# irconde/SSL4POLYP

Hardware: AMD Instinct MI355X
Metric: training-step images/sec/node, ViT-B/16 224^2 (cls fine-tune) (higher is better)
Workload: dtype bf16; 1 GPU; ViT-B/16 classification fine-tune, bs=64/GPU, 224^2, AdamW, random init, finetune mode full (finetune.py:49-91); global_batch=64, parallelism=dp1, launch=eager, lr_schedule=constant

## Files before the change

include/polypmae.h:

```cpp
#ifndef POLYPMAE_H
#define POLYPMAE_H
#include <stddef.h>
#include <stdint.h>

#ifdef __cplusplus
extern "C" {
#endif

enum pm_status { PM_OK = 0, PM_EINVAL = -1, PM_ESHAPE = -2, PM_EARCH = -3, PM_ELAUNCH = -4, PM_EALIGN = -5 };
enum pm_dtype { PM_F32 = 0, PM_BF16 = 1, PM_F16 = 2 };

enum pm_epilogue {
  PM_EPI_STORE = 0,
  PM_EPI_GELU = 1,
  PM_EPI_RESIDUAL = 2,
  PM_EPI_DGELU = 3,
  PM_EPI_ACCUM = 4
};

const char* pm_strerror(int status);
int pm_abi_version(void);

int pm_layernorm_fwd(const float* x, long ldx, const float* gamma, const float* beta, void* y, int out_dtype,
                     float* mean, float* rstd, int M, int D, float eps, void* stream);

int pm_layernorm_bwd(const void* dy, int dy_dtype, const float* x, long ldx, const float* gamma, const float* mean,
                     const float* rstd, const float* dres, long lddres, float* dx, long lddx, void* dx_act,
                     int act_dtype, float* dgamma, float* dbeta, float* dcolsum, int M, int D, void* workspace,
                     size_t ws_bytes, void* stream);

int pm_gemm(const void* A, long lda, int a_kmajor, const void* B, long ldb, int b_kmajor, int in_dtype,
            const float* bias, void* C, long ldc, int c_dtype, int epilogue, void* aux, const float* resid,
            int M, int N, int K, void* stream);

int pm_gemm_ws(const void* A, long lda, int a_kmajor, const void* B, long ldb, int b_kmajor, int in_dtype,
               const float* bias, void* C, long ldc, int c_dtype, int epilogue, void* aux, const float* resid,
               int M, int N, int K, void* workspace, size_t ws_bytes, void* stream);

typedef struct pm_gemm_opts {
  int max_blocks;
  int variant;
} pm_gemm_opts;
int pm_gemm_ex(const void* A, long lda, int a_kmajor, const void* B, long ldb, int b_kmajor, int in_dtype,
               const float* bias, void* C, long ldc, int c_dtype, int epilogue, void* aux, const float* resid,
               int M, int N, int K, void* workspace, size_t ws_bytes, const pm_gemm_opts* opts, void* stream);

typedef struct pm_wgrad_item {
  const void* dY;
  long lddy;
  const void* X;
  long ldx;
  float* dW;
  long lddw;
  int n_out, n_in;
  int accumulate;
  float* dbias;
} pm_wgrad_item;
#define PM_GROUP_WHOLE_K (-1)
int pm_wgrad_group(const pm_wgrad_item* items, int n, int K, int in_dtype, int max_blocks, void* workspace, size_t ws_bytes,
                   void* stream);
size_t pm_wgrad_group_workspace_bytes(const pm_wgrad_item* items, int n, int K, int in_dtype);
int pm_wgrad_group_plan(const pm_wgrad_item* items, int n, int K, int in_dtype, size_t* ws_bytes, int* tiles256,
                        int* k_slices);

int pm_gemm_colsum(const void* A, long lda, int a_kmajor, const void* B, long ldb, int b_kmajor, int in_dtype,
                   const float* bias, void* C, long ldc, int c_dtype, int epilogue, void* aux, const float* resid,
                   float* colsum, int M, int N, int K, void* workspace, size_t ws_bytes, void* stream);

int pm_attention_fwd(const void* qkv, void* out, float* lse, int B, int N, int H, int dh, int dtype, void* stream);
int pm_attention_bwd(const void* qkv, const void* out, const void* dout, const float* lse, float* delta, void* dqkv,
                     int B, int N, int H, int dh, int dtype, void* stream);

int pm_colsum(const void* x, long ldx, int dtype, float* out, int M, int N, void* stream);
int pm_colsum_ws(const void* x, long ldx, int dtype, float* out, int M, int N, void* workspace, size_t ws_bytes,
                 void* stream);

int pm_patch_im2col(const float* imgs, const int* ids_keep, void* cols, long ldcols, int out_dtype, int B, int C, int img,
                    int p, int keep, void* stream);

int pm_pad_cast(const float* src, long lds, void* dst, long ldd, int dst_dtype, int rows, int cols, int rows_pad,
                int cols_pad, void* stream);
int pm_unpad_add(const float* src, long lds, float* dst, long ldd, int rows, int cols, int accumulate, void* stream);

int pm_assemble_tokens(const float* emb, const float* cls, const float* pos, const int* ids_keep, float* x,
                       int B, int keep, int D, void* stream);
int pm_assemble_tokens_bwd(const float* dx, const int* ids_keep, void* demb, int act_dtype, float* dcls, float* dpos,
                           int B, int keep, int D, void* stream);

int pm_mae_noise(float* noise, long n, unsigned long long seed, unsigned int stream_id, void* stream);
int pm_mae_masking(const float* noise, int* ids_shuffle, int* ids_restore, float* mask, int B, int L, int len_keep,
                   void* stream);

int pm_mae_unshuffle(const float* emb, const float* mask_token, const float* dpos, const int* ids_restore, float* out,
                     int B, int L, int keep, int D, void* stream);
int pm_mae_unshuffle_bwd(const float* dout, const int* ids_shuffle, void* demb, int act_dtype, float* dmask_token,
                         int B, int L, int keep, int D, void* workspace, size_t ws_bytes, void* stream);

int pm_mae_loss_fwd(const float* imgs, const float* pred, long ldp, int has_cls_row, float* patch_loss, int B, int C,
                    int img, int p, int norm_pix, void* stream);
int pm_mae_loss_finish(const float* patch_loss, const float* mask, long n, float* sums, float* loss, void* stream);
int pm_mae_loss_bwd(const float* imgs, const float* pred, long ldp, int has_cls_row, const float* mask,
                    const float* sums, const float* dloss, void* dpred, long lddp, int act_dtype, int B, int C, int img,
                    int p, int norm_pix, void* stream);

int pm_gather_rows(const void* src, long ld_bytes, const int* idx, void* dst, int R, long row_bytes, void* stream);
int pm_scatter_rows_zero(const void* src, const int* inv, void* dst, int M, long row_bytes, void* stream);

int pm_cast(const float* src, void* dst, int dst_dtype, long n, void* stream);

int pm_preprocess_u8(const unsigned char* src, const unsigned char* flip_flags, float* dst, int B, int H, int W,
                     float mean_r, float mean_g, float mean_b, float std_r, float std_g, float std_b, void* stream);


int pm_aug_resize_u8(const unsigned char* src, unsigned char* tmp, unsigned char* dst, const int* bounds_x, const int* taps_x,
                     int ksize_x, const int* bounds_y, const int* taps_y, int ksize_y, int B, int Hs, int Ws, int Ho, int Wo,
                     void* stream);

size_t pm_aug_resized_crop_workspace_bytes(int B, int Hs, int Ws, int out);
int pm_aug_resized_crop_u8(const unsigned char* src, const int* box, unsigned char* dst, int bicubic, int B, int Hs, int Ws, int out,
                           void* workspace, size_t ws_bytes, void* stream);
int pm_aug_resized_crop_ragged_u8(const unsigned char* src, const long long* offset, const int* hw, const int* box, unsigned char* dst,
                                  int bicubic, int B, int Hmax, int Wmax, int out, void* workspace, size_t ws_bytes, void* stream);

typedef struct pm_aug_jitter {
  int order[4];
  float brightness, contrast, saturation;
  int hue_shift;
} pm_aug_jitter;
int pm_aug_color_jitter_u8(const unsigned char* src, unsigned char* dst, const pm_aug_jitter* jitter, unsigned long long* lsum,
                           int B, int H, int W, void* stream);

int pm_aug_gaussian_blur_u8(const unsigned char* src, float* tmp, unsigned char* dst, const float* taps, int ksize, int B, int H,
                            int W, void* stream);

typedef struct pm_aug_geom {
  int mode, a0, a1, a2, a3, a4, a5, flips;
} pm_aug_geom;
int pm_aug_geometry_u8(const unsigned char* src, const pm_aug_geom* geom, void* dst, int to_f32, int B, int H, int W, float mean_r,
                       float mean_g, float mean_b, float std_r, float std_g, float std_b, void* stream);

typedef struct pm_aug_boxblur {
  int radius;
  unsigned int ww, fw;
} pm_aug_boxblur;
int pm_aug_pil_gaussian_blur_u8(const unsigned char* src, unsigned char* tmp, unsigned char* dst, const pm_aug_boxblur* prm,
                                int passes, int B, int H, int W, void* stream);
int pm_aug_occlude_u8(unsigned char* img, const int* rects, int B, int H, int W, void* stream);
int pm_aug_jpeg_roundtrip_u8(const unsigned char* src, unsigned char* dst, const int* quality, int B, int H, int W, void* stream);

int pm_jpeg_decode(const unsigned char* entropy, long entropy_bytes, const int* intervals, int n_intervals, const int* frames,
                   int n_frames, const unsigned char* huff, int n_huff, const int* quant, int n_quant, const unsigned char* fallback,
                   long fallback_bytes, const long long* fallback_table, int n_fallback, short* coef, unsigned char* planes,
                   long blocks, long pixels, unsigned char* out, long out_bytes, void* stream);

int pm_jpeg_decode_workspace(int n_intervals, int n_subseq, size_t* bytes);
int pm_jpeg_decode_parallel(const unsigned char* entropy, long entropy_bytes, const int* intervals, int n_intervals, const int* frames,
                            int n_frames, const unsigned char* huff, int n_huff, const int* quant, int n_quant,
                            const unsigned char* fallback, long fallback_bytes, const long long* fallback_table, int n_fallback,
                            short* coef, unsigned char* planes, long blocks, long pixels, unsigned char* out, long out_bytes,
                            const int* subseq, int n_subseq, int sync_rounds, void* workspace, size_t ws_bytes, int* stats,
                            void* stream);

int pm_jpeg_decode_planes(const unsigned char* entropy, long entropy_bytes, const int* intervals, int n_intervals, const int* frames,
                          int n_frames, const unsigned char* huff, int n_huff, const int* quant, int n_quant, short* coef,
                          unsigned char* planes, long blocks, const int* subseq, int n_subseq, int sync_rounds, void* workspace,
                          size_t ws_bytes, int* stats, void* stream);

int pm_jpeg_resized_crop_workspace(int B, int Hmax, int Wmax, int out, size_t* bytes);
int pm_jpeg_resized_crop_u8(const unsigned char* planes, long blocks, const int* frames, int n_frames, const unsigned char* fallback,
                            long fallback_bytes, const long long* fallback_table, int n_fallback, const int* source, const int* hw,
                            const int* box, unsigned char* dst, int bicubic, int B, int Hmax, int Wmax, int out, void* workspace,
                            size_t ws_bytes, void* stream);

typedef struct pm_block_fwd_desc {
  const float* x;
  float* x_mid;
  float* x_out;
  void* ln1;
  float* mean1;
  float* rstd1;
  void* qkv;
  float* lse;
  void* attn;
  void* ln2;
  float* mean2;
  float* rstd2;
  void* h_pre;
  void* h_act;
  const float *norm1_w, *norm1_b, *norm2_w, *norm2_b;
  const void *qkv_w, *proj_w, *fc1_w, *fc2_w;
  const float *qkv_b, *proj_b, *fc1_b, *fc2_b;
  int rows, samples, N, D, Hd, heads;
  int dtype;
  int gemm_variant;
  float eps;
} pm_block_fwd_desc;
int pm_vit_block_fwd(const pm_block_fwd_desc* d, void* stream);

typedef struct pm_block_bwd_desc {
  const float* x_in;
  const float* x_mid;
  const void *ln1, *qkv, *attn, *ln2, *h_pre, *h_act;
  const float *mean1, *rstd1, *mean2, *rstd2, *lse;
  const float *norm1_w, *norm2_w;
  const void *qkv_w, *proj_w, *fc1_w, *fc2_w;
  const float* dx;
  const void* dx_act;
  float* dmid;
  void* dmid_act;
  float* din;
  void* din_act;
  void *d_hidden, *d_qkv, *d_ln, *d_attn;
  float* delta;
  float *g_norm1_w, *g_norm1_b, *g_norm2_w, *g_norm2_b;
  float *g_qkv_w, *g_proj_w, *g_fc1_w, *g_fc2_w;
  float *g_qkv_b, *g_proj_b, *g_fc1_b, *g_below_bias;
  void* ws_ln;
  size_t ws_ln_bytes;
  void* ws_group;
  size_t ws_group_bytes;
  void *side_stream, *ev_join, *ev_fork, *ev_done;
  int samples, N, D, Hd, heads, dtype, gemm_variant, group_blocks, accumulate;
  int two_groups;
  void *side_stream2, *ev_fork2, *ev_done2;
} pm_block_bwd_desc;
int pm_vit_block_bwd(const pm_block_bwd_desc* d, void* stream);

int pm_vit_head_fwd(const float* x, int N, int pool, const float* gamma, const float* beta, const float* W,
                    const float* bias, float* feat, float* xhat_mean, float* mean, float* rstd, float* logits, int B, int D,
                    int n_class, float eps, void* stream);
int pm_vit_head_bwd(const float* dlogits, const float* dfeat, const float* x, int N, int pool, const float* gamma,
                    const float* W, const float* feat, const float* xhat_mean, const float* mean, const float* rstd,
                    float* dx, void* dx_act, int act_dtype, float* dW, float* dbias, float* dgamma, float* dbeta, int B,
                    int D, int n_class, void* stream);
int pm_cls_head_fwd(const float* x, int N, const float* gamma, const float* beta, const float* W, const float* bias,
                    float* xn, float* mean, float* rstd, float* logits, int B, int D, int n_class, float eps,
                    void* stream);
int pm_cls_head_bwd(const float* dlogits, const float* x, int N, const float* gamma, const float* W, const float* xn,
                    const float* mean, const float* rstd, float* dx, void* dx_act, int act_dtype, float* dW,
                    float* dbias, float* dgamma, float* dbeta, int B, int D, int n_class, void* stream);

int pm_supervised_loss_fwd(const float* logits, const long long* targets, const float* pos_weight,
                           const float* class_weights, float* loss, float* dlogits, int B, int n_class, void* stream);
int pm_scale(const float* x, const float* scale, float* out, long n, void* stream);

int pm_dgelu(const void* dy, const void* pre, void* out, int dtype, long n, void* stream);

int pm_adamw(float* p, const float* g, float* m, float* v, void* shadow, int shadow_dtype, long n, float lr,
             float beta1, float beta2, float eps, float weight_decay, int step, float grad_scale, void* stream);

int pm_adamw_tick(float* hyper, int n_groups, void* stream);
int pm_adamw_dev(float* p, const float* g, float* m, float* v, void* shadow, int shadow_dtype, long n,
                 const float* hyper, void* stream);

int pm_loss_scale_update(float* state, const float* stats, float* hyper, int n_groups, float growth_factor,
                         float backoff_factor, int growth_interval, void* stream);

int pm_grad_stats(const float* g, long n, float* out, void* stream);

enum pm_ws_kind { PM_WS_LAYERNORM_BWD = 1, PM_WS_COLSUM = 2, PM_WS_GEMM_COLSUM = 3, PM_WS_UNSHUFFLE_BWD = 4 };
size_t pm_gemm_workspace_bytes(int a_kmajor, int b_kmajor, int in_dtype, int M, int N, int K, const pm_gemm_opts* opts);
size_t pm_workspace_bytes(int kind, int M, int N);

typedef struct pm_comm pm_comm;
int pm_comm_unique_id(void* id128);
int pm_comm_create(pm_comm** out, const void* id128, int rank, int world);
int pm_comm_world(const pm_comm* c, int* rank, int* world);
int pm_comm_allreduce_f32(pm_comm* c, float* base, const long* lo, const long* hi, int n_buckets, void* stream);
int pm_comm_destroy(pm_comm* c);

int pm_boot_metrics_workspace(int N, int M, int R, int K, int C, size_t* bytes);
int pm_boot_metrics(const double* score, const int* order, const unsigned char* label, const int* cluster, const int* draws,
                    const double* tau, double* out, int N, int M, int R, int K, int C, int sorted_ready, void* workspace,
                    size_t ws_bytes, void* stream);

#ifdef __cplusplus
}
#endif
#endif
```

ssl4polyp_amd/_lib.py:

```python
from __future__ import annotations

import ctypes
import os
from ctypes import c_char_p, c_float, c_int, c_long, c_void_p

PM_F32, PM_BF16, PM_F16 = 0, 1, 2
EPI_STORE, EPI_GELU, EPI_RESIDUAL, EPI_DGELU, EPI_ACCUM = 0, 1, 2, 3, 4

_HERE = os.path.dirname(os.path.abspath(__file__))
LIB_PATH = os.environ.get("POLYPMAE_LIB") or os.path.join(_HERE, "lib", "libpolypmae.so")

P, I, L, F = c_void_p, c_int, c_long, c_float

SIGNATURES = {
    "pm_layernorm_fwd": [P, L, P, P, P, I, P, P, I, I, F, P],
    "pm_layernorm_bwd": [P, I, P, L, P, P, P, P, L, P, L, P, I, P, P, P, I, I, P, ctypes.c_size_t, P],
    "pm_vit_block_fwd": [P, P],
    "pm_vit_block_bwd": [P, P],
    "pm_gemm": [P, L, I, P, L, I, I, P, P, L, I, I, P, P, I, I, I, P],
    "pm_gemm_ws": [P, L, I, P, L, I, I, P, P, L, I, I, P, P, I, I, I, P, ctypes.c_size_t, P],
    "pm_gemm_ex": [P, L, I, P, L, I, I, P, P, L, I, I, P, P, I, I, I, P, ctypes.c_size_t, P, P],
    "pm_wgrad_group": [P, I, I, I, I, P, ctypes.c_size_t, P],
    "pm_wgrad_group_plan": [P, I, I, I, P, P, P],
    "pm_gemm_colsum": [P, L, I, P, L, I, I, P, P, L, I, I, P, P, P, I, I, I, P, ctypes.c_size_t, P],
    "pm_attention_fwd": [P, P, P, I, I, I, I, I, P],
    "pm_attention_bwd": [P, P, P, P, P, P, I, I, I, I, I, P],
    "pm_colsum": [P, L, I, P, I, I, P],
    "pm_colsum_ws": [P, L, I, P, I, I, P, ctypes.c_size_t, P],
    "pm_patch_im2col": [P, P, P, L, I, I, I, I, I, I, P],
    "pm_pad_cast": [P, L, P, L, I, I, I, I, I, P],
    "pm_unpad_add": [P, L, P, L, I, I, I, P],
    "pm_assemble_tokens": [P, P, P, P, P, I, I, I, P],
    "pm_assemble_tokens_bwd": [P, P, P, I, P, P, I, I, I, P],
    "pm_mae_noise": [P, L, ctypes.c_ulonglong, ctypes.c_uint, P],
    "pm_mae_masking": [P, P, P, P, I, I, I, P],
    "pm_mae_unshuffle": [P, P, P, P, P, I, I, I, I, P],
    "pm_mae_unshuffle_bwd": [P, P, P, I, P, I, I, I, I, P, ctypes.c_size_t, P],
    "pm_mae_loss_fwd": [P, P, L, I, P, I, I, I, I, I, P],
    "pm_mae_loss_finish": [P, P, L, P, P, P],
    "pm_mae_loss_bwd": [P, P, L, I, P, P, P, P, L, I, I, I, I, I, I, P],
    "pm_cast": [P, P, I, L, P],
    "pm_gather_rows": [P, L, P, P, I, L, P],
    "pm_scatter_rows_zero": [P, P, P, I, L, P],
    "pm_preprocess_u8": [P, P, P, I, I, I, F, F, F, F, F, F, P],
    "pm_aug_resize_u8": [P, P, P, P, P, I, P, P, I, I, I, I, I, I, P],
    "pm_aug_resized_crop_u8": [P, P, P, I, I, I, I, I, P, ctypes.c_size_t, P],
    "pm_aug_resized_crop_ragged_u8": [P, P, P, P, P, I, I, I, I, I, P, ctypes.c_size_t, P],
    "pm_aug_color_jitter_u8": [P, P, P, P, I, I, I, P],
    "pm_aug_gaussian_blur_u8": [P, P, P, P, I, I, I, I, P],
    "pm_aug_geometry_u8": [P, P, P, I, I, I, I, F, F, F, F, F, F, P],
    "pm_aug_pil_gaussian_blur_u8": [P, P, P, P, I, I, I, I, P],
    "pm_aug_occlude_u8": [P, P, I, I, I, P],
    "pm_aug_jpeg_roundtrip_u8": [P, P, P, I, I, I, P],
    "pm_jpeg_decode": [P, L, P, I, P, I, P, I, P, I, P, L, P, I, P, P, L, L, P, L, P],
    "pm_jpeg_decode_parallel": [P, L, P, I, P, I, P, I, P, I, P, L, P, I, P, P, L, L, P, L, P, I, I, P, ctypes.c_size_t, P, P],
    "pm_jpeg_decode_workspace": [I, I, P],
    "pm_jpeg_decode_planes": [P, L, P, I, P, I, P, I, P, I, P, P, L, P, I, I, P, ctypes.c_size_t, P, P],
    "pm_jpeg_resized_crop_workspace": [I, I, I, I, P],
    "pm_jpeg_resized_crop_u8": [P, L, P, I, P, L, P, I, P, P, P, P, I, I, I, I, I, P, ctypes.c_size_t, P],
    "pm_comm_unique_id": [P],
    "pm_comm_create": [P, P, I, I],
    "pm_comm_world": [P, P, P],
    "pm_comm_allreduce_f32": [P, P, P, P, I, P],
    "pm_comm_destroy": [P],
    "pm_vit_head_fwd": [P, I, I, P, P, P, P, P, P, P, P, P, I, I, I, F, P],
    "pm_vit_head_bwd": [P, P, P, I, I, P, P, P, P, P, P, P, P, I, P, P, P, P, I, I, I, P],
    "pm_supervised_loss_fwd": [P, P, P, P, P, P, I, I, P],
    "pm_scale": [P, P, P, L, P],
    "pm_cls_head_fwd": [P, I, P, P, P, P, P, P, P, P, I, I, I, F, P],
    "pm_cls_head_bwd": [P, P, I, P, P, P, P, P, P, P, I, P, P, P, P, I, I, I, P],
    "pm_adamw": [P, P, P, P, P, I, L, F, F, F, F, F, I, F, P],
    "pm_adamw_tick": [P, I, P],
    "pm_adamw_dev": [P, P, P, P, P, I, L, P, P],
    "pm_grad_stats": [P, L, P, P],
    "pm_loss_scale_update": [P, P, P, I, F, F, I, P],
    "pm_dgelu": [P, P, P, I, L, P],
    "pm_boot_metrics_workspace": [I, I, I, I, I, P],
    "pm_boot_metrics": [P, P, P, P, P, P, P, I, I, I, I, I, I, P, ctypes.c_size_t, P],
}

ABI_VERSION = 14
PM_GROUP_WHOLE_K = -1

WS_LAYERNORM_BWD, WS_COLSUM, WS_GEMM_COLSUM, WS_UNSHUFFLE_BWD = 1, 2, 3, 4


class GemmOpts(ctypes.Structure):
    _fields_ = [("max_blocks", c_int), ("variant", c_int)]


class WgradItem(ctypes.Structure):
    _fields_ = [("dY", c_void_p), ("lddy", c_long), ("X", c_void_p), ("ldx", c_long), ("dW", c_void_p), ("lddw", c_long),
                ("n_out", c_int), ("n_in", c_int), ("accumulate", c_int), ("dbias", c_void_p)]


class BlockBwdDesc(ctypes.Structure):
    _fields_ = ([(n, c_void_p) for n in ("x_in", "x_mid", "ln1", "qkv", "attn", "ln2", "h_pre", "h_act", "mean1", "rstd1", "mean2",
                                        "rstd2", "lse", "norm1_w", "norm2_w", "qkv_w", "proj_w", "fc1_w", "fc2_w", "dx", "dx_act",
                                        "dmid", "dmid_act", "din", "din_act", "d_hidden", "d_qkv", "d_ln", "d_attn", "delta",
                                        "g_norm1_w", "g_norm1_b", "g_norm2_w", "g_norm2_b", "g_qkv_w", "g_proj_w", "g_fc1_w",
                                        "g_fc2_w", "g_qkv_b", "g_proj_b", "g_fc1_b", "g_below_bias")] +
                [("ws_ln", c_void_p), ("ws_ln_bytes", ctypes.c_size_t), ("ws_group", c_void_p), ("ws_group_bytes", ctypes.c_size_t)] +
                [(n, c_void_p) for n in ("side_stream", "ev_join", "ev_fork", "ev_done")] +
                [(n, c_int) for n in ("samples", "N", "D", "Hd", "heads", "dtype", "gemm_variant", "group_blocks", "accumulate",
                                      "two_groups")] +
                [(n, c_void_p) for n in ("side_stream2", "ev_fork2", "ev_done2")])


class BlockFwdDesc(ctypes.Structure):
    _fields_ = ([(n, c_void_p) for n in ("x", "x_mid", "x_out", "ln1", "mean1", "rstd1", "qkv", "lse", "attn", "ln2", "mean2",
                                        "rstd2", "h_pre", "h_act", "norm1_w", "norm1_b", "norm2_w", "norm2_b", "qkv_w", "proj_w",
                                        "fc1_w", "fc2_w", "qkv_b", "proj_b", "fc1_b", "fc2_b")] +
                [(n, c_int) for n in ("rows", "samples", "N", "D", "Hd", "heads", "dtype", "gemm_variant")] +
                [("eps", ctypes.c_float)])


PM_EINVAL, PM_ESHAPE, PM_EALIGN = -1, -2, -5
_lib = None


class PolypMaeError(RuntimeError):
    pass


def load():
    global _lib
    if _lib is not None:
        return _lib
    if not os.path.exists(LIB_PATH):
        raise PolypMaeError(
            f"{LIB_PATH} not found: build it with `python -c 'import __graft_entry__ as g; g.build()'`. "
            "There is no CPU/eager fallback for the MI355X hot path.")
    lib = ctypes.CDLL(LIB_PATH)
    lib.pm_strerror.restype = c_char_p
    lib.pm_strerror.argtypes = [c_int]
    lib.pm_abi_version.restype = c_int
    lib.pm_abi_version.argtypes = []
    if lib.pm_abi_version() != ABI_VERSION:
        raise PolypMaeError(f"{LIB_PATH} has ABI version {lib.pm_abi_version()}, this package binds version {ABI_VERSION}: "
                            "rebuild with `python -c 'import __graft_entry__ as g; g.build(force=True)'`")
    lib.pm_gemm_workspace_bytes.restype = ctypes.c_size_t
    lib.pm_gemm_workspace_bytes.argtypes = [I, I, I, I, I, I, P]
    lib.pm_workspace_bytes.restype = ctypes.c_size_t
    lib.pm_workspace_bytes.argtypes = [I, I, I]
    lib.pm_aug_resized_crop_workspace_bytes.restype = ctypes.c_size_t
    lib.pm_aug_resized_crop_workspace_bytes.argtypes = [I, I, I, I]
    lib.pm_wgrad_group_workspace_bytes.restype = ctypes.c_size_t
    lib.pm_wgrad_group_workspace_bytes.argtypes = [P, I, I, I]
    for name, argtypes in SIGNATURES.items():
        fn = getattr(lib, name)
        fn.restype = c_int
        fn.argtypes = argtypes
    _lib = lib
    return lib


def check(status: int, what: str) -> None:
    if status != 0:
        raise PolypMaeError(f"{what} failed: {load().pm_strerror(status).decode()} (status {status})")


def dtype_code(torch_dtype) -> int:
    import torch

    if torch_dtype == torch.float32:
        return PM_F32
    if torch_dtype == torch.bfloat16:
        return PM_BF16
    if torch_dtype == torch.float16:
        return PM_F16
    raise PolypMaeError(f"unsupported dtype {torch_dtype}")
```

ssl4polyp_amd/csrc/pm_block.hip:

```cpp
#include "pm_common.h"

extern "C" int pm_vit_block_fwd(const pm_block_fwd_desc* d, void* stream) {
  if (!d) return PM_EINVAL;
  if (!d->x || !d->x_mid || !d->x_out || !d->ln1 || !d->qkv || !d->attn || !d->ln2 || !d->h_act) return PM_EINVAL;
  if (d->rows <= 0 || d->samples <= 0 || d->N <= 0 || d->rows != d->samples * d->N) return PM_ESHAPE;
  if (d->D <= 0 || d->Hd <= 0 || d->heads <= 0 || (d->D % d->heads)) return PM_ESHAPE;
  if (d->dtype != PM_BF16 && d->dtype != PM_F16 && d->dtype != PM_F32) return PM_EINVAL;
  const int M = d->rows, D = d->D, Hd = d->Hd, dt = d->dtype;
  pm_gemm_opts opts;
  opts.max_blocks = 0;
  opts.variant = d->gemm_variant;
  int st;
  if ((st = pm_layernorm_fwd(d->x, D, d->norm1_w, d->norm1_b, d->ln1, dt, d->mean1, d->rstd1, M, D, d->eps, stream))) return st;
  if ((st = pm_gemm_ex(d->ln1, D, 0, d->qkv_w, D, 0, dt, d->qkv_b, d->qkv, 3 * D, dt, PM_EPI_STORE, nullptr, nullptr, M, 3 * D,
                       D, nullptr, 0, &opts, stream)))
    return st;
  if ((st = pm_attention_fwd(d->qkv, d->attn, d->lse, d->samples, d->N, d->heads, D / d->heads, dt, stream))) return st;
  if ((st = pm_gemm_ex(d->attn, D, 0, d->proj_w, D, 0, dt, d->proj_b, d->x_mid, D, PM_F32, PM_EPI_RESIDUAL, nullptr, d->x, M, D,
                       D, nullptr, 0, &opts, stream)))
    return st;
  if ((st = pm_layernorm_fwd(d->x_mid, D, d->norm2_w, d->norm2_b, d->ln2, dt, d->mean2, d->rstd2, M, D, d->eps, stream))) return st;
  if ((st = pm_gemm_ex(d->ln2, D, 0, d->fc1_w, D, 0, dt, d->fc1_b, d->h_act, Hd, dt, PM_EPI_GELU, d->h_pre, nullptr, M, Hd, D,
                       nullptr, 0, &opts, stream)))
    return st;
  return pm_gemm_ex(d->h_act, Hd, 0, d->fc2_w, Hd, 0, dt, d->fc2_b, d->x_out, D, PM_F32, PM_EPI_RESIDUAL, nullptr, d->x_mid, M, D,
                    Hd, nullptr, 0, &opts, stream);
}

extern "C" int pm_vit_block_bwd(const pm_block_bwd_desc* d, void* stream) {
  if (!d) return PM_EINVAL;
  if (!d->x_in || !d->x_mid || !d->ln1 || !d->qkv || !d->attn || !d->ln2 || !d->h_pre || !d->h_act || !d->dx || !d->dx_act ||
      !d->dmid || !d->dmid_act || !d->din || !d->din_act || !d->d_hidden || !d->d_qkv || !d->d_ln || !d->d_attn || !d->delta)
    return PM_EINVAL;
  if (!d->g_qkv_w || !d->g_proj_w || !d->g_fc1_w || !d->g_fc2_w || !d->side_stream || !d->ev_fork || !d->ev_done) return PM_EINVAL;
  if (d->samples <= 0 || d->N <= 0 || d->D <= 0 || d->Hd <= 0 || d->heads <= 0 || (d->D % d->heads)) return PM_ESHAPE;
  if (d->dtype != PM_BF16 && d->dtype != PM_F16 && d->dtype != PM_F32) return PM_EINVAL;
  const int M = d->samples * d->N, D = d->D, Hd = d->Hd, dt = d->dtype;
  hipStream_t main = pm_stream(stream), side = pm_stream(d->side_stream);
  pm_gemm_opts opts;
  opts.max_blocks = 0;
  opts.variant = d->gemm_variant;
  int st;
  pm_wgrad_item it[4];
  size_t ws_need = 0;
  {
    const void* dys[4] = {d->dx_act, d->d_hidden, d->dmid_act, d->d_qkv};
    const void* xs[4] = {d->h_act, d->ln2, d->attn, d->ln1};
    float* dws[4] = {d->g_fc2_w, d->g_fc1_w, d->g_proj_w, d->g_qkv_w};
    float* dbs[4] = {nullptr, d->g_fc1_b, nullptr, d->g_qkv_b};
    const int n_out[4] = {D, Hd, D, 3 * D}, n_in[4] = {Hd, D, D, D};
    const int acc_bit[4] = {3, 2, 1, 0};
    for (int j = 0; j < 4; ++j) {
      it[j].dY = dys[j]; it[j].lddy = n_out[j]; it[j].X = xs[j]; it[j].ldx = n_in[j]; it[j].dW = dws[j]; it[j].lddw = n_in[j];
      it[j].n_out = n_out[j]; it[j].n_in = n_in[j]; it[j].accumulate = (d->accumulate >> acc_bit[j]) & 1; it[j].dbias = dbs[j];
    }
    if ((st = pm_wgrad_group_plan(it, 4, M, dt, &ws_need, nullptr, nullptr))) return st;
  }
  bool two = false;
  if (d->two_groups) {
    if (!d->side_stream2 || !d->ev_fork2 || !d->ev_done2) return PM_EINVAL;
    int slices = 0;
    if ((st = pm_wgrad_group_plan(it, 2, M, dt, nullptr, nullptr, &slices))) return st;
    if ((st = pm_wgrad_group_plan(it + 2, 2, M, dt, nullptr, nullptr, nullptr))) return st;
    two = slices == 1;
  }
  if (!two && ws_need > 0 && (!d->ws_group || d->ws_group_bytes < ws_need)) return PM_EINVAL;
  hipStream_t side2 = two ? pm_stream(d->side_stream2) : nullptr;
  if (d->ev_join && hipStreamWaitEvent(main, (hipEvent_t)d->ev_join, 0) != hipSuccess) return PM_ELAUNCH;
  if ((st = pm_gemm_ex(d->dx_act, D, 0, d->fc2_w, Hd, 1, dt, nullptr, d->d_hidden, Hd, dt, PM_EPI_DGELU, (void*)d->h_pre, nullptr, M,
                       Hd, D, nullptr, 0, &opts, stream)))
    return st;
  if (two) {
    if (hipEventRecord((hipEvent_t)d->ev_fork, main) != hipSuccess) return PM_ELAUNCH;
    if (hipStreamWaitEvent(side, (hipEvent_t)d->ev_fork, 0) != hipSuccess) return PM_ELAUNCH;
    if ((st = pm_wgrad_group(it, 2, M, dt, d->group_blocks, nullptr, 0, d->side_stream))) return st;
    if (hipEventRecord((hipEvent_t)d->ev_done, side) != hipSuccess) return PM_ELAUNCH;
  }
  if ((st = pm_gemm_ex(d->d_hidden, Hd, 0, d->fc1_w, D, 1, dt, nullptr, d->d_ln, D, dt, PM_EPI_STORE, nullptr, nullptr, M, D, Hd,
                       nullptr, 0, &opts, stream)))
    return st;
  if ((st = pm_layernorm_bwd(d->d_ln, dt, d->x_mid, D, d->norm2_w, d->mean2, d->rstd2, d->dx, D, d->dmid, D, d->dmid_act, dt,
                             d->g_norm2_w, d->g_norm2_b, d->g_proj_b, M, D, d->ws_ln, d->ws_ln_bytes, stream)))
    return st;
  if ((st = pm_gemm_ex(d->dmid_act, D, 0, d->proj_w, D, 1, dt, nullptr, d->d_attn, D, dt, PM_EPI_STORE, nullptr, nullptr, M, D, D,
                       nullptr, 0, &opts, stream)))
    return st;
  if ((st = pm_attention_bwd(d->qkv, d->attn, d->d_attn, d->lse, d->delta, d->d_qkv, d->samples, d->N, d->heads, D / d->heads, dt,
                             stream)))
    return st;
  if (two) {
    if (hipEventRecord((hipEvent_t)d->ev_fork2, main) != hipSuccess) return PM_ELAUNCH;
    if (hipStreamWaitEvent(side2, (hipEvent_t)d->ev_fork2, 0) != hipSuccess) return PM_ELAUNCH;
    if ((st = pm_wgrad_group(it + 2, 2, M, dt, PM_GROUP_WHOLE_K, nullptr, 0, d->side_stream2))) return st;
    if (hipEventRecord((hipEvent_t)d->ev_done2, side2) != hipSuccess) return PM_ELAUNCH;
  } else {
    if (hipEventRecord((hipEvent_t)d->ev_fork, main) != hipSuccess) return PM_ELAUNCH;
    if (hipStreamWaitEvent(side, (hipEvent_t)d->ev_fork, 0) != hipSuccess) return PM_ELAUNCH;
    if ((st = pm_wgrad_group(it, 4, M, dt, d->group_blocks, d->ws_group, d->ws_group_bytes, d->side_stream))) return st;
    if (hipEventRecord((hipEvent_t)d->ev_done, side) != hipSuccess) return PM_ELAUNCH;
  }
  if ((st = pm_gemm_ex(d->d_qkv, 3 * D, 0, d->qkv_w, D, 1, dt, nullptr, d->d_ln, D, dt, PM_EPI_STORE, nullptr, nullptr, M, D, 3 * D,
                       nullptr, 0, &opts, stream)))
    return st;
  return pm_layernorm_bwd(d->d_ln, dt, d->x_in, D, d->norm1_w, d->mean1, d->rstd1, d->dmid, D, d->din, D, d->din_act, dt,
                          d->g_norm1_w, d->g_norm1_b, d->g_below_bias, M, D, d->ws_ln, d->ws_ln_bytes, stream);
}
```

ssl4polyp_amd/csrc/pm_layernorm.hip:

```cpp
#include "pm_common.h"

namespace {

constexpr int kMaxD = 1280;

template <typename TOut, int NV>
__global__ __launch_bounds__(256) void ln_fwd_kernel(const float* __restrict__ x, long ldx, const float* __restrict__ gamma,
                                                     const float* __restrict__ beta, TOut* __restrict__ y,
                                                     float* __restrict__ mean_out, float* __restrict__ rstd_out, int M,
                                                     int D, float eps) {
  constexpr int kMaxVec = NV;
  const int lane = threadIdx.x & 63;
  const int wave = threadIdx.x >> 6;
  const int nvec = D >> 2;
  for (long row = (long)blockIdx.x * 4 + wave; row < M; row += (long)gridDim.x * 4) {
    const float* xr = x + row * ldx;
    f32x4 v[kMaxVec];
    float s = 0.f;
#pragma unroll
    for (int i = 0; i < kMaxVec; ++i) {
      const int c = lane + 64 * i;
      if (c < nvec) {
        v[i] = *reinterpret_cast<const f32x4*>(xr + 4 * c);
        s += (v[i][0] + v[i][1]) + (v[i][2] + v[i][3]);
      }
    }
    const float mean = wave_sum(s) / (float)D;
    float q = 0.f;
#pragma unroll
    for (int i = 0; i < kMaxVec; ++i) {
      const int c = lane + 64 * i;
      if (c < nvec) {
#pragma unroll
        for (int e = 0; e < 4; ++e) {
          const float d = v[i][e] - mean;
          q += d * d;
        }
      }
    }
    const float rstd = rsqrtf(wave_sum(q) / (float)D + eps);
    if (lane == 0) {
      mean_out[row] = mean;
      rstd_out[row] = rstd;
    }
    TOut* yr = y + row * (long)D;
#pragma unroll
    for (int i = 0; i < kMaxVec; ++i) {
      const int c = lane + 64 * i;
      if (c < nvec) {
        const f32x4 g = *reinterpret_cast<const f32x4*>(gamma + 4 * c);
        const f32x4 b = *reinterpret_cast<const f32x4*>(beta + 4 * c);
        f32x4 o;
#pragma unroll
        for (int e = 0; e < 4; ++e) o[e] = (v[i][e] - mean) * rstd * g[e] + b[e];
        store4<TOut>(yr + 4 * c, o);
      }
    }
  }
}

template <typename TDy, typename TAct, int NV>
__global__ __launch_bounds__(256) void ln_bwd_kernel(const TDy* __restrict__ dy, const float* __restrict__ x, long ldx,
                                                     const float* __restrict__ gamma, const float* __restrict__ mean,
                                                     const float* __restrict__ rstd, const float* __restrict__ dres,
                                                     long lddres, float* __restrict__ dx, long lddx,
                                                     TAct* __restrict__ dx_act, float* __restrict__ dgamma,
                                                     float* __restrict__ dbeta, float* __restrict__ dcolsum,
                                                     float* __restrict__ partials, int M, int D) {
  __shared__ float red[3][4][256 + 4];
  constexpr int kMaxVec = NV;
  const int lane = threadIdx.x & 63;
  const int wave = threadIdx.x >> 6;
  const int nvec = D >> 2;
  f32x4 g[kMaxVec];
  f32x4 acc_g[kMaxVec], acc_b[kMaxVec], acc_c[kMaxVec];
#pragma unroll
  for (int i = 0; i < kMaxVec; ++i) {
    const int c = lane + 64 * i;
    const f32x4 z = {0.f, 0.f, 0.f, 0.f};
    g[i] = (c < nvec) ? *reinterpret_cast<const f32x4*>(gamma + 4 * c) : z;
    acc_g[i] = z;
    acc_b[i] = z;
    acc_c[i] = z;
  }
  const float invD = 1.0f / (float)D;
  const long stride = (long)gridDim.x * 4;
  for (long row0 = (long)blockIdx.x * 4 + wave; row0 < M; row0 += 2 * stride) {
    long rows[2] = {row0, row0 + stride};
    const bool valid[2] = {true, rows[1] < M};
    if (!valid[1]) rows[1] = row0;
    float mu[2], rs[2], s1[2] = {0.f, 0.f}, s2[2] = {0.f, 0.f};
    f32x4 xh[2][kMaxVec], dv[2][kMaxVec], dr[2][kMaxVec];
#pragma unroll
    for (int u = 0; u < 2; ++u) {
      mu[u] = mean[rows[u]];
      rs[u] = rstd[rows[u]];
#pragma unroll
      for (int i = 0; i < kMaxVec; ++i) {
        const int c = lane + 64 * i;
        if (c < nvec) {
          xh[u][i] = *reinterpret_cast<const f32x4*>(x + rows[u] * ldx + 4 * c);
          dv[u][i] = load4<TDy>(dy + rows[u] * (long)D + 4 * c);
          if (dres) dr[u][i] = *reinterpret_cast<const f32x4*>(dres + rows[u] * lddres + 4 * c);
        }
      }
    }
#pragma unroll
    for (int u = 0; u < 2; ++u) {
      const float live = valid[u] ? 1.0f : 0.0f;
#pragma unroll
      for (int i = 0; i < kMaxVec; ++i) {
        const int c = lane + 64 * i;
        if (c < nvec) {
#pragma unroll
          for (int e = 0; e < 4; ++e) {
            xh[u][i][e] = (xh[u][i][e] - mu[u]) * rs[u];
            const float gg = dv[u][i][e] * g[i][e];
            s1[u] += gg;
            s2[u] += gg * xh[u][i][e];
            acc_g[i][e] += live * dv[u][i][e] * xh[u][i][e];
            acc_b[i][e] += live * dv[u][i][e];
          }
        }
      }
    }
    float c1[2], c2[2];
#pragma unroll
    for (int u = 0; u < 2; ++u) {
      c1[u] = s1[u];
      c2[u] = s2[u];
    }
#pragma unroll
    for (int o = 32; o > 0; o >>= 1) {
      c1[0] += __shfl_xor(c1[0], o, 64);
      c1[1] += __shfl_xor(c1[1], o, 64);
      c2[0] += __shfl_xor(c2[0], o, 64);
      c2[1] += __shfl_xor(c2[1], o, 64);
    }
#pragma unroll
    for (int u = 0; u < 2; ++u) {
      if (!valid[u]) continue;
      const float k1 = c1[u] * invD, k2 = c2[u] * invD;
#pragma unroll
      for (int i = 0; i < kMaxVec; ++i) {
        const int c = lane + 64 * i;
        if (c < nvec) {
          f32x4 o;
#pragma unroll
          for (int e = 0; e < 4; ++e) o[e] = rs[u] * (dv[u][i][e] * g[i][e] - k1 - xh[u][i][e] * k2);
          if (dres) o += dr[u][i];
          *reinterpret_cast<f32x4*>(dx + rows[u] * lddx + 4 * c) = o;
          if (dx_act) store4<TAct>(dx_act + rows[u] * (long)D + 4 * c, o);
#pragma unroll
          for (int e = 0; e < 4; ++e) acc_c[i][e] += o[e];
        }
      }
    }
  }
#pragma unroll
  for (int i = 0; i < kMaxVec; ++i) {
    const int c = lane + 64 * i;
    __syncthreads();
#pragma unroll
    for (int e = 0; e < 4; ++e) {
      red[0][wave][lane * 4 + e] = acc_g[i][e];
      red[1][wave][lane * 4 + e] = acc_b[i][e];
      red[2][wave][lane * 4 + e] = acc_c[i][e];
    }
    __syncthreads();
    if (wave < 3 && c < nvec) {
      float* dst = wave == 0 ? dgamma : (wave == 1 ? dbeta : dcolsum);
      if (dst) {
        f32x4 t;
#pragma unroll
        for (int e = 0; e < 4; ++e)
          t[e] = (red[wave][0][lane * 4 + e] + red[wave][1][lane * 4 + e]) +
                 (red[wave][2][lane * 4 + e] + red[wave][3][lane * 4 + e]);
        if (partials) {
          *reinterpret_cast<f32x4*>(partials + ((long)blockIdx.x * 3 + wave) * D + 4 * c) = t;
        } else {
#pragma unroll
          for (int e = 0; e < 4; ++e) atomicAdd(dst + 4 * c + e, t[e]);
        }
      }
    }
  }
}

__global__ __launch_bounds__(1024) void ln_bwd_reduce_kernel(const float* __restrict__ partials, float* dgamma, float* dbeta,
                                                             float* dcolsum, int nblocks, int D) {
  __shared__ float red[16][64];
  const int lane = threadIdx.x & 63, rg = threadIdx.x >> 6;
  const int d = blockIdx.x * 64 + lane;
  const int v = blockIdx.y;
  float* dst = v == 0 ? dgamma : (v == 1 ? dbeta : dcolsum);
  if (!dst) return;
  float s0 = 0.f;
  if (d < D) s0 = strided_sum<16>(partials + (long)v * D + d, 3L * D, rg, 16, nblocks);
  red[rg][lane] = s0;
  __syncthreads();
  if (rg == 0 && d < D) {
    float t = 0.f;
#pragma unroll
    for (int g = 0; g < 16; ++g) t += red[g][lane];
    dst[d] += t;
  }
}

inline int ln_grid(int M) {
  int g = (M + 3) / 4;
  return g < 1 ? 1 : (g > 1024 ? 1024 : g);
}

}

extern "C" int pm_layernorm_fwd(const float* x, long ldx, const float* gamma, const float* beta, void* y, int out_dtype,
                                float* mean, float* rstd, int M, int D, float eps, void* stream) {
  if (!x || !gamma || !beta || !y || !mean || !rstd) return PM_EINVAL;
  if (M <= 0 || D <= 0 || D > kMaxD || (D & 3) || (ldx & 3)) return PM_ESHAPE;
  const int grid = (M + 3) / 4 > 4096 ? 4096 : (M + 3) / 4;
#define PM_LN_FWD(TO, NV) \
  hipLaunchKernelGGL((ln_fwd_kernel<TO, NV>), dim3(grid), dim3(256), 0, pm_stream(stream), x, ldx, gamma, beta, (TO*)y, mean, rstd, M, D, eps)
  PM_DISPATCH_ACT(out_dtype, T, {
    if (D <= 1024) PM_LN_FWD(T, 4); else PM_LN_FWD(T, 5);
  });
#undef PM_LN_FWD
  return pm_check_launch();
}

extern "C" int pm_layernorm_bwd(const void* dy, int dy_dtype, const float* x, long ldx, const float* gamma,
                                const float* mean, const float* rstd, const float* dres, long lddres, float* dx,
                                long lddx, void* dx_act, int act_dtype, float* dgamma, float* dbeta, float* dcolsum,
                                int M, int D, void* workspace, size_t ws_bytes, void* stream) {
  if (!dy || !x || !gamma || !mean || !rstd || !dx) return PM_EINVAL;
  if (M <= 0 || D <= 0 || D > kMaxD || (D & 3) || (ldx & 3) || (lddx & 3) || (dres && (lddres & 3))) return PM_ESHAPE;
  if (dx_act && act_dtype != dy_dtype) return PM_EINVAL;
  int grid = (M + 3) / 4;
  float* partials = nullptr;
  const bool want_sums = dgamma || dbeta || dcolsum;
  if (want_sums && workspace && ws_bytes >= (size_t)64 * 3 * D * sizeof(float)) {
    int cap = (int)(ws_bytes / ((size_t)3 * D * sizeof(float)));
    if (cap > 1024) cap = 1024;
    if (grid > cap) grid = cap;
    partials = reinterpret_cast<float*>(workspace);
  } else if (grid > 256) {
    grid = 256;
  }
  if (grid < 1) grid = 1;
  hipStream_t s = pm_stream(stream);
  const int nv = (D + 255) / 256;
#define PM_LN_BWD(TD, NV)                                                                                               \
  hipLaunchKernelGGL((ln_bwd_kernel<TD, TD, NV>), dim3(grid), dim3(256), 0, s, (const TD*)dy, x, ldx, gamma, mean, rstd, \
                     dres, lddres, dx, lddx, (TD*)dx_act, dgamma, dbeta, dcolsum, partials, M, D)
  PM_DISPATCH_ACT(dy_dtype, T, {
    if (nv == 1) PM_LN_BWD(T, 1); else if (nv == 2) PM_LN_BWD(T, 2); else if (nv == 3) PM_LN_BWD(T, 3);
    else if (nv == 4) PM_LN_BWD(T, 4); else PM_LN_BWD(T, 5);
  });
#undef PM_LN_BWD
  if (partials)
    hipLaunchKernelGGL(ln_bwd_reduce_kernel, dim3((D + 63) / 64, 3), dim3(1024), 0, s, partials, dgamma, dbeta, dcolsum, grid, D);
  return pm_check_launch();
}
```

ssl4polyp_amd/engine.py:

```python
from __future__ import annotations

from dataclasses import dataclass
from typing import Callable, Dict, List, Optional, Sequence, Tuple

import contextlib
import ctypes
import os

import torch

from . import _lib
from ._lib import EPI_ACCUM, EPI_DGELU, EPI_GELU, EPI_RESIDUAL, EPI_STORE, PM_BF16, PM_F16, PM_F32

LN_EPS = 1e-6

BLOCK_PARAM_NAMES = (
    "norm1.weight", "norm1.bias", "attn.qkv.weight", "attn.qkv.bias", "attn.proj.weight", "attn.proj.bias",
    "norm2.weight", "norm2.bias", "mlp.fc1.weight", "mlp.fc1.bias", "mlp.fc2.weight", "mlp.fc2.bias")


def _ptr(t: Optional[torch.Tensor]) -> Optional[int]:
    return None if t is None else t.data_ptr()


_raw_stream = getattr(torch._C, "_cuda_getCurrentRawStream", None)
_cur_device = getattr(torch._C, "_cuda_getDevice", None)


def _stream() -> int:
    if _raw_stream is not None:
        return _raw_stream(_cur_device())
    return torch.cuda.current_stream().cuda_stream


_STREAMS: Dict[Tuple[int, str], "torch.cuda.Stream"] = {}
MERGE_AUX_SIDE2 = os.environ.get("PM_MERGE_AUX_SIDE2", "1") == "1"


def _shared_stream(device, role: str):
    dev = torch.device(device)
    key = (dev.index if dev.index is not None else torch.cuda.current_device(), role)
    st = _STREAMS.get(key)
    if st is None:
        st = _STREAMS[key] = torch.cuda.Stream(device=dev)
    return st


def reserve_streams(device) -> None:
    dev = torch.device(device)
    torch.zeros(1, device=dev)
    for role in ("aux0", "side") + (() if MERGE_AUX_SIDE2 else ("side2",)):
        with torch.cuda.stream(_shared_stream(dev, role)):
            torch.zeros(1, device=dev)
    torch.cuda.synchronize(dev)


PRECISIONS = {"bf16": (torch.bfloat16, PM_BF16), "fp16": (torch.float16, PM_F16), "fp32": (torch.float32, PM_F32)}


class Kernels:

    def __init__(self, precision: str, eps: float = LN_EPS):
        self.eps = float(eps)
        if precision not in PRECISIONS:
            raise ValueError("precision must be 'bf16', 'fp16' or 'fp32'")
        self.lib = _lib.load()
        self.precision = precision
        self.act_dtype, self.act = PRECISIONS[precision]

    def layernorm_fwd(self, x, gamma, beta, y, mean, rstd, M, D):
        _lib.check(self.lib.pm_layernorm_fwd(_ptr(x), D, _ptr(gamma), _ptr(beta), _ptr(y), _lib.dtype_code(y.dtype),
                                             _ptr(mean), _ptr(rstd), M, D, self.eps, _stream()), "pm_layernorm_fwd")

    def layernorm_bwd(self, dy, x, gamma, mean, rstd, dres, dx, dx_act, dgamma, dbeta, dcolsum, M, D):
        ws = self._scratch("_ws_ln", self._need(("ln", M, D), lambda: self.lib.pm_workspace_bytes(_lib.WS_LAYERNORM_BWD, M, D)),
                           x.device)
        _lib.check(self.lib.pm_layernorm_bwd(_ptr(dy), _lib.dtype_code(dy.dtype), _ptr(x), D, _ptr(gamma), _ptr(mean),
                                             _ptr(rstd), _ptr(dres), D, _ptr(dx), D, _ptr(dx_act), self.act,
                                             _ptr(dgamma), _ptr(dbeta), _ptr(dcolsum), M, D, _ptr(ws), ws.numel(), _stream()),
                   "pm_layernorm_bwd")

    SPLIT_FORWARD = int(os.environ.get("PM_SPLIT_FWD", "2"))
    WGRAD_BLOCKS = int(os.environ.get("PM_WGRAD_BLOCKS", "128"))
    FUSE_COLSUM = os.environ.get("PM_FUSE_COLSUM", "0") == "1"
    TWO_GROUPS = os.environ.get("PM_TWO_GROUPS", "1") == "1"
    TIME_BLOCK_EVENTS = False
    gemm_variant = int(os.environ.get("PM_GEMM_VARIANT", "0"))

    def _need(self, key, query) -> int:
        cache = self.__dict__.setdefault("_need_cache", {})
        n = cache.get(key)
        if n is None:
            n = cache[key] = int(query())
        return n

    def _scratch(self, name: str, nbytes: int, device) -> torch.Tensor:
        ws = getattr(self, name, None)
        if ws is None or ws.device != device or ws.numel() < nbytes:
            if ws is not None and ws.device == device:
                torch.cuda.synchronize(device)
            ws = torch.empty(max(nbytes, 1 << 16), dtype=torch.uint8, device=device)
            setattr(self, name, ws)
        return ws

    def aux_stream(self, device, j: int = 0):
        return _shared_stream(device, f"aux{j}")

    def side_stream(self, device):
        st = getattr(self, "_side", None)
        if st is None or st.device != device:
            st = self._side = _shared_stream(device, "side")
        return st

    def side_stream2(self, device):
        st = getattr(self, "_side2", None)
        if st is None or st.device != device:
            st = self._side2 = _shared_stream(device, "aux0" if MERGE_AUX_SIDE2 else "side2")
        return st

    def _opts(self, wgrad: bool):
        o = self.__dict__.get("_opts_cache")
        if o is None or o[0] != (self.WGRAD_BLOCKS, self.gemm_variant):
            key = (self.WGRAD_BLOCKS, self.gemm_variant)
            o = self._opts_cache = (key, _lib.GemmOpts(self.WGRAD_BLOCKS, self.gemm_variant), _lib.GemmOpts(0, self.gemm_variant))
        return o[1] if wgrad else o[2]

    def gemm(self, A, lda, a_kmajor, B, ldb, b_kmajor, bias, C, ldc, epilogue, M, N, K, aux=None, resid=None, colsum=None,
             ws_name="_ws"):
        in_dtype = _lib.dtype_code(A.dtype)
        if _lib.dtype_code(B.dtype) != in_dtype:
            raise _lib.PolypMaeError("pm_gemm: operand dtypes differ")
        if colsum is not None:
            ws = self._colsum_workspace(A.device, M, N, True)
            _lib.check(self.lib.pm_gemm_colsum(_ptr(A), lda, int(a_kmajor), _ptr(B), ldb, int(b_kmajor), in_dtype, _ptr(bias),
                                               _ptr(C), ldc, _lib.dtype_code(C.dtype), epilogue, _ptr(aux), _ptr(resid),
                                               _ptr(colsum), M, N, K, _ptr(ws), ws.numel(), _stream()), "pm_gemm_colsum")
            return
        wgrad = bool(a_kmajor and b_kmajor)
        opts = self._opts(wgrad)
        ws = None
        if wgrad:
            need = self._need(("gemm", in_dtype, M, N, K, opts.max_blocks, opts.variant),
                              lambda: self.lib.pm_gemm_workspace_bytes(1, 1, in_dtype, M, N, K, ctypes.byref(opts)))
            ws = self._scratch(ws_name, need, A.device)
        _lib.check(self.lib.pm_gemm_ex(_ptr(A), lda, int(a_kmajor), _ptr(B), ldb, int(b_kmajor), in_dtype, _ptr(bias),
                                       _ptr(C), ldc, _lib.dtype_code(C.dtype), epilogue, _ptr(aux), _ptr(resid), M, N, K,
                                       _ptr(ws), ws.numel() if ws is not None else 0, ctypes.byref(opts), _stream()), "pm_gemm")

    def linear_fwd(self, x, W, bias, out, M, N, K, epilogue=EPI_STORE, aux=None, resid=None):
        self.gemm(x, K, 0, W, K, 0, bias, out, N, epilogue, M, N, K, aux=aux, resid=resid)

    def linear_dgrad(self, dy, W, dx, M, N_out, K_in, epilogue=EPI_STORE, aux=None, colsum=None):
        self.gemm(dy, N_out, 0, W, K_in, 1, None, dx, K_in, epilogue, M, K_in, N_out, aux=aux, colsum=colsum)

    DEFER_JOIN = os.environ.get("PM_DEFER_JOIN", "1") != "0"
    BLOCK_CALLS = os.environ.get("PM_BLOCK_CALLS", "1") != "0"
    GROUP_WGRAD = os.environ.get("PM_GROUP_WGRAD", "1") != "0"
    GROUP_BLOCKS = int(os.environ.get("PM_GROUP_BLOCKS", "0"))
    GROUP_BLOCKS_SLICED = int(os.environ.get("PM_GROUP_BLOCKS_SLICED", "0"))
    GROUP_MIN_TILES = int(os.environ.get("PM_GROUP_MIN_TILES", "64"))
    GROUP_BIAS = os.environ.get("PM_GROUP_BIAS", "1") != "0"
    GROUP_SPLIT = os.environ.get("PM_GROUP_SPLIT", "1") != "0"
    UNGROUP_TAIL = int(os.environ.get("PM_UNGROUP_TAIL", "1"))

    def wgrad_group(self, items, K, whole_k: bool = False) -> bool:
        n = len(items)
        arr = (_lib.WgradItem * n)()
        for j, (dy, x, dW, acc, *rest) in enumerate(items):
            n_out, n_in = dW.shape
            arr[j] = _lib.WgradItem(_ptr(dy), n_out, _ptr(x), n_in, _ptr(dW), n_in, n_out, n_in, int(bool(acc)),
                                    _ptr(rest[0]) if rest and rest[0] is not None else None)
        dt = _lib.dtype_code(items[0][0].dtype)
        key = ("group", K, dt, tuple((tuple(it[2].shape), len(it) > 4 and it[4] is not None) for it in items))
        need = 0 if whole_k else self._need(key, lambda: self.lib.pm_wgrad_group_workspace_bytes(arr, n, K, dt))
        ws = self._scratch("_ws_group", need, items[0][0].device) if need else None
        blocks = _lib.PM_GROUP_WHOLE_K if whole_k else (self.GROUP_BLOCKS_SLICED if need else self.GROUP_BLOCKS)
        st = self.lib.pm_wgrad_group(arr, n, K, dt, blocks, _ptr(ws), ws.numel() if ws is not None else 0, _stream())
        if st == _lib.PM_ESHAPE:
            return False
        _lib.check(st, "pm_wgrad_group")
        return True

    def can_group_wgrad(self, K: int, dims) -> bool:
        if not self.GROUP_WGRAD:
            return False
        key = ("can_group", K, self.act, tuple(dims), self.GROUP_MIN_TILES, self.GROUP_SPLIT)
        cache = self.__dict__.setdefault("_need_cache", {})
        hit = cache.get(key)
        if hit is not None:
            return hit
        n = len(dims)
        arr = (_lib.WgradItem * n)()
        for j, (o, i) in enumerate(dims):
            arr[j] = _lib.WgradItem(64, o, 64, i, 64, i, o, i, 0, None)
        tiles, slices = ctypes.c_int(0), ctypes.c_int(0)
        st = self.lib.pm_wgrad_group_plan(arr, n, K, self.act, None, ctypes.byref(tiles), ctypes.byref(slices))
        ok = st == 0 and (tiles.value >= self.GROUP_MIN_TILES or (self.GROUP_SPLIT and slices.value > 1))
        cache[key] = ok
        return ok

    def two_launch_group(self, K: int, dims) -> bool:
        if not self.TWO_GROUPS:
            return False
        key = ("two_launch", K, self.act, tuple(dims))
        cache = self.__dict__.setdefault("_need_cache", {})
        hit = cache.get(key)
        if hit is None:
            ok = True
            for first, part in ((True, dims[:2]), (False, dims[2:])):
                arr = (_lib.WgradItem * 2)()
                for j, (o, i) in enumerate(part):
                    arr[j] = _lib.WgradItem(64, o, 64, i, 64, i, o, i, 0, None)
                slices = ctypes.c_int(0)
                st = self.lib.pm_wgrad_group_plan(arr, 2, K, self.act, None, None, ctypes.byref(slices))
                ok = ok and st == 0 and (slices.value == 1 or not first)
            hit = cache[key] = ok
        return hit

    def linear_wgrad(self, dy, x, dW, M, N_out, K_in, accumulate, ws_name="_ws"):
        self.gemm(dy, N_out, 1, x, K_in, 1, None, dW, K_in, EPI_ACCUM if accumulate else EPI_STORE, N_out, K_in, M, ws_name=ws_name)

    def _colsum_workspace(self, device, M: int, N: int, fused: bool = False):
        on_side = getattr(self, "_side", None) is not None and torch.cuda.current_stream() == self._side
        kind = _lib.WS_GEMM_COLSUM if fused else _lib.WS_COLSUM
        need = self._need(("cs", kind, M, N), lambda: self.lib.pm_workspace_bytes(kind, M, N))
        return self._scratch("_ws_cs_side" if on_side else "_ws_cs_main", need, device)

    def colsum(self, x, out, M, N):
        ws = self._colsum_workspace(x.device, M, N)
        _lib.check(self.lib.pm_colsum_ws(_ptr(x), N, _lib.dtype_code(x.dtype), _ptr(out), M, N, _ptr(ws), ws.numel(),
                                         _stream()), "pm_colsum")

    def attention_fwd(self, qkv, out, lse, B, N, H, dh):
        _lib.check(self.lib.pm_attention_fwd(_ptr(qkv), _ptr(out), _ptr(lse), B, N, H, dh, self.act, _stream()),
                   "pm_attention_fwd")

    def attention_bwd(self, qkv, out, dout, lse, delta, dqkv, B, N, H, dh):
        _lib.check(self.lib.pm_attention_bwd(_ptr(qkv), _ptr(out), _ptr(dout), _ptr(lse), _ptr(delta), _ptr(dqkv), B, N,
                                             H, dh, self.act, _stream()), "pm_attention_bwd")

    def gather_rows(self, src: torch.Tensor, idx: torch.Tensor, out: Optional[torch.Tensor] = None) -> torch.Tensor:
        rows = src if src.ndim == 2 else src.view(-1, 1)
        dst = out if out is not None else torch.empty(idx.numel(), rows.shape[1], dtype=src.dtype, device=src.device)
        rb = rows.shape[1] * src.element_size()
        _lib.check(self.lib.pm_gather_rows(_ptr(rows), rb, _ptr(idx), _ptr(dst), idx.numel(), rb, _stream()), "pm_gather_rows")
        return dst if src.ndim == 2 else dst.view(-1)

    def scatter_rows_zero(self, src: torch.Tensor, inv: torch.Tensor, dst: torch.Tensor) -> None:
        _lib.check(self.lib.pm_scatter_rows_zero(_ptr(src), _ptr(inv), _ptr(dst), dst.shape[0], dst.shape[1] * dst.element_size(),
                                                 _stream()), "pm_scatter_rows_zero")

    SPARSE_TOP = os.environ.get("PM_SPARSE_TOP", "1") != "0"

    def cast(self, src, dst):
        _lib.check(self.lib.pm_cast(_ptr(src), _ptr(dst), _lib.dtype_code(dst.dtype), src.numel(), _stream()), "pm_cast")

    @staticmethod
    def padded_k(K: int) -> int:
        return K if K % 64 == 0 else (K + 63) // 64 * 64

    def pad_cast(self, src: torch.Tensor, rows_pad: int, cols_pad: int) -> torch.Tensor:
        rows, cols = src.shape
        dst = torch.empty(rows_pad, cols_pad, dtype=self.act_dtype, device=src.device)
        _lib.check(self.lib.pm_pad_cast(_ptr(src), cols, _ptr(dst), cols_pad, self.act, rows, cols, rows_pad, cols_pad, _stream()),
                   "pm_pad_cast")
        return dst

    def unpad_add(self, src: torch.Tensor, dst: torch.Tensor, accumulate: bool) -> None:
        rows, cols = dst.shape
        _lib.check(self.lib.pm_unpad_add(_ptr(src), src.shape[1], _ptr(dst), cols, rows, cols, 1 if accumulate else 0, _stream()),
                   "pm_unpad_add")


@dataclass
class StackGeom:
    dim: int
    heads: int
    depth: int
    hidden: int

    @property
    def dh(self) -> int:
        return self.dim // self.heads


class BlockWorkspace:

    def __init__(self, g: StackGeom, B: int, N: int, act_dtype, dev):
        M, D, Hd = B * N, g.dim, g.hidden
        f32 = torch.float32
        e = lambda *s, dt=act_dtype: torch.empty(*s, dtype=dt, device=dev)
        self.mean1, self.rstd1 = e(M, dt=f32), e(M, dt=f32)
        self.ln1 = e(M, D)
        self.qkv = e(M, 3 * D)
        self.lse = e(B * g.heads * N, dt=f32)
        self.attn = e(M, D)
        self.x_mid = e(M, D, dt=f32)
        self.mean2, self.rstd2 = e(M, dt=f32), e(M, dt=f32)
        self.ln2 = e(M, D)
        self.h_pre = e(M, Hd)
        self.h_act = e(M, Hd)
        self.x_out = e(M, D, dt=f32)


class StackWorkspace:

    def __init__(self, g: StackGeom, B: int, N: int, act_dtype, dev, training: bool):
        self.B, self.N, self.M = B, N, B * N
        M, D, Hd = self.M, g.dim, g.hidden
        f32 = torch.float32
        nblk = g.depth if training else min(g.depth, 2)
        self.blocks = [BlockWorkspace(g, B, N, act_dtype, dev) for _ in range(nblk)]
        self.training = training
        if training:
            e = lambda *s, dt=act_dtype: torch.empty(*s, dtype=dt, device=dev)
            self.d_hidden = [e(M, Hd), e(M, Hd)]
            self.d_qkv = [e(M, 3 * D), e(M, 3 * D)]
            self.d_ln = e(M, D)
            self.d_attn = e(M, D)
            self.delta = e(B * g.heads * N, dt=f32)
            self.dx = [e(M, D, dt=f32), e(M, D, dt=f32)]
            self.dx_act = [e(M, D) for _ in range(5)]

    def block(self, i: int) -> BlockWorkspace:
        return self.blocks[i if self.training else i % len(self.blocks)]


class BlockStack:

    def __init__(self, k: Kernels, g: StackGeom):
        self.k, self.g = k, g

    def forward(self, ws: StackWorkspace, x_in: torch.Tensor, W: Sequence[Dict[str, torch.Tensor]],
                before_block: Optional[Callable[[int], None]] = None, keep_from: int = 0, cls_top: bool = False) -> torch.Tensor:
        k, g = self.k, self.g
        if not ws.training:
            keep_from = g.depth
        cls_top = cls_top and ws.N > 1 and g.depth >= 1
        B, N, M, D, Hd = ws.B, ws.N, ws.M, g.dim, g.hidden
        if cls_top and x_in.is_cuda:
            self.top_compact(ws, g, k.act_dtype, x_in.device)
        main = torch.cuda.current_stream() if x_in.is_cuda else None
        nparts = min(k.SPLIT_FORWARD, B)
        split = nparts > 1 and main is not None and not torch.cuda.is_current_stream_capturing()
        if split:
            auxs = [k.aux_stream(x_in.device, j) for j in range(nparts - 1)]
            ev = torch.cuda.Event()
            ev.record(main)
            for aux in auxs:
                aux.wait_event(ev)
            cuts = [B * j // nparts for j in range(nparts + 1)]
            parts = [((main if j == 0 else auxs[j - 1]), cuts[j], cuts[j + 1]) for j in range(nparts)]
        else:
            parts = [(None, 0, B)]
        fast = k.BLOCK_CALLS and x_in.is_cuda
        if fast:
            lib = k.lib
            cache = ws.__dict__.setdefault("_fwd_descs", {})
            raw = [(st.cuda_stream if st is not None and st is not main else None) for st, _, _ in parts]
        x = x_in
        for i in range(g.depth):
            if before_block is not None:
                if split:
                    before_block(i, also=auxs)
                else:
                    before_block(i)
            bw, p = ws.block(i), W[i]
            if cls_top and i == g.depth - 1:
                x = self._top_block_forward_cls(ws, bw, p, x, parts, main, i >= keep_from)
                continue
            if fast:
                for j, (st, b0, b1) in enumerate(parts):
                    key = (b0, b1, x.data_ptr(), p["attn.qkv.weight"].data_ptr(), p["norm1.weight"].data_ptr(), k.gemm_variant,
                           i >= keep_from)
                    ent = cache.get((i, j))
                    if ent is None or ent[0] != key:
                        ent = cache[(i, j)] = (key, self._fwd_desc(ws, bw, p, x, b0, b1, keep=i >= keep_from))
                    _lib.check(lib.pm_vit_block_fwd(ctypes.byref(ent[1]), raw[j] if raw[j] is not None else _stream()),
                               "pm_vit_block_fwd")
                x = bw.x_out
                continue
            for st, b0, b1 in parts:
                r0, r1, Bh = b0 * N, b1 * N, b1 - b0
                Mh = r1 - r0
                h0, h1 = b0 * g.heads * N, b1 * g.heads * N
                with (torch.cuda.stream(st) if st is not None and st is not main else contextlib.nullcontext()):
                    xs = x[r0:r1]
                    k.layernorm_fwd(xs, p["norm1.weight"], p["norm1.bias"], bw.ln1[r0:r1], bw.mean1[r0:r1], bw.rstd1[r0:r1],
                                    Mh, D)
                    k.linear_fwd(bw.ln1[r0:r1], p["attn.qkv.weight"], p["attn.qkv.bias"], bw.qkv[r0:r1], Mh, 3 * D, D)
                    k.attention_fwd(bw.qkv[r0:r1], bw.attn[r0:r1], bw.lse[h0:h1], Bh, N, g.heads, g.dh)
                    k.linear_fwd(bw.attn[r0:r1], p["attn.proj.weight"], p["attn.proj.bias"], bw.x_mid[r0:r1], Mh, D, D,
                                 EPI_RESIDUAL, resid=xs)
                    k.layernorm_fwd(bw.x_mid[r0:r1], p["norm2.weight"], p["norm2.bias"], bw.ln2[r0:r1], bw.mean2[r0:r1],
                                    bw.rstd2[r0:r1], Mh, D)
                    k.linear_fwd(bw.ln2[r0:r1], p["mlp.fc1.weight"], p["mlp.fc1.bias"], bw.h_act[r0:r1], Mh, Hd, D, EPI_GELU,
                                 aux=bw.h_pre[r0:r1] if i >= keep_from else None)
                    k.linear_fwd(bw.h_act[r0:r1], p["mlp.fc2.weight"], p["mlp.fc2.bias"], bw.x_out[r0:r1], Mh, D, Hd,
                                 EPI_RESIDUAL, resid=bw.x_mid[r0:r1])
            x = bw.x_out
        if split:
            for aux in auxs:
                ev = torch.cuda.Event()
                ev.record(aux)
                main.wait_event(ev)
        return x

    @staticmethod
    def top_compact(ws: StackWorkspace, g: StackGeom, act_dtype, dev) -> dict:
        tc = ws.__dict__.get("_top_c")
        if tc is None:
            B, N, D, Hd, f32 = ws.B, ws.N, g.dim, g.hidden, torch.float32
            e = lambda *s, dt=act_dtype: torch.empty(*s, dtype=dt, device=dev)
            rows = torch.arange(B, dtype=torch.int32, device=dev) * N
            inv = torch.full((B * N,), -1, dtype=torch.int32, device=dev)
            inv[rows.long()] = torch.arange(B, dtype=torch.int32, device=dev)
            tc = ws.__dict__["_top_c"] = dict(
                rows=rows, inv=inv, x=e(B, D, dt=f32), attn=e(B, D), x_mid=e(B, D, dt=f32), ln2=e(B, D), mean2=e(B, dt=f32),
                rstd2=e(B, dt=f32), h_pre=e(B, Hd), h_act=e(B, Hd), x_out=e(B, D, dt=f32), dx=e(B, D, dt=f32), dx_act=e(B, D))
        return tc

    def _top_block_forward_cls(self, ws, bw, p, x, parts, main, keep: bool) -> torch.Tensor:
        k, g = self.k, self.g
        N, D, Hd = ws.N, g.dim, g.hidden
        tc = self.top_compact(ws, g, k.act_dtype, x.device)
        for st, b0, b1 in parts:
            r0, r1, Bh = b0 * N, b1 * N, b1 - b0
            Mh = r1 - r0
            h0, h1 = b0 * g.heads * N, b1 * g.heads * N
            with (torch.cuda.stream(st) if st is not None and st is not main else contextlib.nullcontext()):
                xs = x[r0:r1]
                k.layernorm_fwd(xs, p["norm1.weight"], p["norm1.bias"], bw.ln1[r0:r1], bw.mean1[r0:r1], bw.rstd1[r0:r1], Mh, D)
                k.linear_fwd(bw.ln1[r0:r1], p["attn.qkv.weight"], p["attn.qkv.bias"], bw.qkv[r0:r1], Mh, 3 * D, D)
                k.attention_fwd(bw.qkv[r0:r1], bw.attn[r0:r1], bw.lse[h0:h1], Bh, N, g.heads, g.dh)
                idx = tc["rows"][b0:b1]
                k.gather_rows(x.view(-1, D), idx, out=tc["x"][b0:b1])
                k.gather_rows(bw.attn.view(-1, D), idx, out=tc["attn"][b0:b1])
                k.linear_fwd(tc["attn"][b0:b1], p["attn.proj.weight"], p["attn.proj.bias"], tc["x_mid"][b0:b1], Bh, D, D, EPI_RESIDUAL,
                             resid=tc["x"][b0:b1])
                k.layernorm_fwd(tc["x_mid"][b0:b1], p["norm2.weight"], p["norm2.bias"], tc["ln2"][b0:b1], tc["mean2"][b0:b1],
                                tc["rstd2"][b0:b1], Bh, D)
                k.linear_fwd(tc["ln2"][b0:b1], p["mlp.fc1.weight"], p["mlp.fc1.bias"], tc["h_act"][b0:b1], Bh, Hd, D, EPI_GELU,
                             aux=tc["h_pre"][b0:b1] if keep else None)
                k.linear_fwd(tc["h_act"][b0:b1], p["mlp.fc2.weight"], p["mlp.fc2.bias"], tc["x_out"][b0:b1], Bh, D, Hd, EPI_RESIDUAL,
                             resid=tc["x_mid"][b0:b1])
        return tc["x_out"]

    def _fwd_desc(self, ws: StackWorkspace, bw: BlockWorkspace, p, x: torch.Tensor, b0: int, b1: int, keep: bool = True):
        k, g = self.k, self.g
        N, D, Hd = ws.N, g.dim, g.hidden
        r0, h0 = b0 * N, b0 * g.heads * N
        a = lambda t, row, width: t.data_ptr() + row * width * t.element_size()
        v = lambda t: t.data_ptr() if t is not None else None
        return _lib.BlockFwdDesc(
            a(x, r0, D), a(bw.x_mid, r0, D), a(bw.x_out, r0, D), a(bw.ln1, r0, D), a(bw.mean1, r0, 1), a(bw.rstd1, r0, 1),
            a(bw.qkv, r0, 3 * D), a(bw.lse, h0, 1), a(bw.attn, r0, D), a(bw.ln2, r0, D), a(bw.mean2, r0, 1), a(bw.rstd2, r0, 1),
            a(bw.h_pre, r0, Hd) if keep else None, a(bw.h_act, r0, Hd),
            v(p["norm1.weight"]), v(p["norm1.bias"]), v(p["norm2.weight"]), v(p["norm2.bias"]),
            v(p["attn.qkv.weight"]), v(p["attn.proj.weight"]), v(p["mlp.fc1.weight"]), v(p["mlp.fc2.weight"]),
            v(p["attn.qkv.bias"]), v(p["attn.proj.bias"]), v(p["mlp.fc1.bias"]), v(p["mlp.fc2.bias"]),
            (b1 - b0) * N, b1 - b0, N, D, Hd, g.heads, k.act, k.gemm_variant, k.eps)

    def _bwd_desc(self, ws, bw, p, gr, xin, dx, dx_act, dmid, dmid_act, din, din_act, d_hidden, d_qkv, below_bias, acc, side, main):
        k, g = self.k, self.g
        M, D, Hd = ws.M, g.dim, g.hidden
        v = lambda t: t.data_ptr() if t is not None else None
        ws_ln = k._scratch("_ws_ln", k._need(("ln", M, D), lambda: k.lib.pm_workspace_bytes(_lib.WS_LAYERNORM_BWD, M, D)), dx.device)
        items = (_lib.WgradItem * 4)()
        for j, (n_out, n_in, bias) in enumerate(((D, Hd, False), (Hd, D, True), (D, D, False), (3 * D, D, True))):
            items[j] = _lib.WgradItem(64, n_out, 64, n_in, 64, n_in, n_out, n_in, 0, 64 if bias else None)
        need = k._need(("groupws", M, k.act, D, Hd), lambda: k.lib.pm_wgrad_group_workspace_bytes(items, 4, M, k.act))
        ws_group = k._scratch("_ws_group", need, dx.device) if need else None
        mk = lambda: torch.cuda.Event(enable_timing=bool(k.TIME_BLOCK_EVENTS))
        ev_fork, ev_done = mk(), mk()
        ev_fork.record(main)
        ev_done.record(main)
        two = not need and k.two_launch_group(M, ((D, Hd), (Hd, D), (D, D), (3 * D, D)))
        ev_fork2 = ev_done2 = side2 = None
        if two:
            side2 = k.side_stream2(dx.device)
            ev_fork2, ev_done2 = mk(), mk()
            ev_fork2.record(main)
            ev_done2.record(main)
        desc = _lib.BlockBwdDesc(
            v(xin), v(bw.x_mid), v(bw.ln1), v(bw.qkv), v(bw.attn), v(bw.ln2), v(bw.h_pre), v(bw.h_act), v(bw.mean1), v(bw.rstd1),
            v(bw.mean2), v(bw.rstd2), v(bw.lse), v(p["norm1.weight"]), v(p["norm2.weight"]), v(p["attn.qkv.weight"]),
            v(p["attn.proj.weight"]), v(p["mlp.fc1.weight"]), v(p["mlp.fc2.weight"]), v(dx), v(dx_act), v(dmid), v(dmid_act), v(din),
            v(din_act), v(d_hidden), v(d_qkv), v(ws.d_ln), v(ws.d_attn), v(ws.delta),
            v(gr["norm1.weight"]), v(gr["norm1.bias"]), v(gr["norm2.weight"]), v(gr["norm2.bias"]), v(gr["attn.qkv.weight"]),
            v(gr["attn.proj.weight"]), v(gr["mlp.fc1.weight"]), v(gr["mlp.fc2.weight"]), v(gr["attn.qkv.bias"]),
            v(gr["attn.proj.bias"]), v(gr["mlp.fc1.bias"]), v(below_bias),
            v(ws_ln), ws_ln.numel(), v(ws_group), ws_group.numel() if ws_group is not None else 0,
            side.cuda_stream, None, ev_fork.cuda_event, ev_done.cuda_event,
            ws.B, ws.N, D, Hd, g.heads, k.act, k.gemm_variant, k.GROUP_BLOCKS_SLICED if need else k.GROUP_BLOCKS, acc,
            int(two), side2.cuda_stream if two else None, ev_fork2.cuda_event if two else None, ev_done2.cuda_event if two else None)
        return desc, (ev_done, ev_done2) if two else (ev_done,), (ev_fork, ev_fork2, ws_ln, ws_group)

    def backward(self, ws: StackWorkspace, x_in: torch.Tensor, W, G, dx: torch.Tensor, dx_act: torch.Tensor,
                 last_bias_grad_done: bool, trainable: Sequence[bool], need_input_grad: bool,
                 accumulate: Callable[[str, int], bool], on_block_done: Optional[Callable[[int], None]] = None,
                 prev_bias_grad: Optional[torch.Tensor] = None,
                 ends_pass: bool = True, defer_join: bool = False,
                 sparse_top: Optional[Tuple[torch.Tensor, torch.Tensor]] = None) -> Tuple[Optional[torch.Tensor], Optional[torch.Tensor]]:
        k, g = self.k, self.g
        B, N, M, D, Hd = ws.B, ws.N, ws.M, g.dim, g.hidden
        lowest = min([i for i, t in enumerate(trainable) if t], default=g.depth)
        main = torch.cuda.current_stream()
        pending: Dict[int, Tuple[torch.cuda.Event, ...]] = {}

        def join(down_to: int):
            for j in sorted((j for j in pending if j >= down_to), reverse=True):
                for ev in pending.pop(j):
                    main.wait_event(ev)

        fast = (k.BLOCK_CALLS and k.GROUP_BIAS and not k.FUSE_COLSUM and dx.is_cuda and
                not torch.cuda.is_current_stream_capturing())
        bcache = ws.__dict__.setdefault("_bwd_descs", {})
        ptr_of = lambda t: t.data_ptr() if t is not None else 0
        for i in reversed(range(g.depth)):
            if i < lowest and not need_input_grad:
                join(0)
                return None, None
            bw, p, gr, tr = ws.block(i), W[i], G[i], trainable[i]
            xin = x_in if i == 0 else ws.block(i - 1).x_out
            need_dx_in = need_input_grad or i > lowest
            o = i & 1
            dmid, din = ws.dx[o], ws.dx[o ^ 1]
            d_hidden, d_qkv = ws.d_hidden[o], ws.d_qkv[o]
            pin = next((j for j in range(5) if dx_act is ws.dx_act[j]), 4)
            dmid_act, din_act = ws.dx_act[(pin + 1) % 5], ws.dx_act[(pin + 2) % 5]
            join(i + 2)
            if i == g.depth - 1 and sparse_top is not None:
                if tr and ws.B % 8:
                    raise _lib.PolypMaeError("the cls-row top block needs a batch that is a multiple of 8 to train (16-byte k-major rows)")
                below_bias = (G[i - 1]["mlp.fc2.bias"] if trainable[i - 1] else None) if i > 0 else prev_bias_grad
                ev_last = self._top_block_sparse(ws, bw, p, gr, xin, dx, dx_act, sparse_top, last_bias_grad_done, dmid, din, din_act,
                                                 d_qkv, below_bias, lambda n: accumulate(n, i), main, on_block_done, i, tr)
                if ev_last is not None:
                    pending[i] = ev_last
                dx, dx_act = din, din_act
                continue
            if i == g.depth - 1 and not last_bias_grad_done and tr:
                k.colsum(dx, gr["mlp.fc2.bias"], M, D)
            side = k.side_stream(main.device) if tr else None

            def fork():
                ev = torch.cuda.Event()
                ev.record(main)
                side.wait_event(ev)

            grouped = tr and (not ends_pass or i - lowest >= k.UNGROUP_TAIL) and k.can_group_wgrad(M, ((D, Hd), (Hd, D), (D, D), (3 * D, D)))
            if grouped and fast:
                below_bias = (G[i - 1]["mlp.fc2.bias"] if trainable[i - 1] else None) if i > 0 else prev_bias_grad
                acc = (int(accumulate("attn.qkv.weight", i)) | int(accumulate("attn.proj.weight", i)) << 1 |
                       int(accumulate("mlp.fc1.weight", i)) << 2 | int(accumulate("mlp.fc2.weight", i)) << 3)
                key = (dx.data_ptr(), dx_act.data_ptr(), xin.data_ptr(), gr["attn.qkv.weight"].data_ptr(),
                       p["attn.qkv.weight"].data_ptr(), gr["norm1.weight"].data_ptr(),
                       below_bias.data_ptr() if below_bias is not None else 0, acc, k.gemm_variant, k.GROUP_BLOCKS, k.GROUP_BLOCKS_SLICED, k.TWO_GROUPS, k.TIME_BLOCK_EVENTS,
                       ptr_of(k.__dict__.get("_ws_ln")), ptr_of(k.__dict__.get("_ws_group")))
                ent = bcache.get(i)
                if ent is None or ent[0] != key:
                    ent = bcache[i] = (key,) + self._bwd_desc(ws, bw, p, gr, xin, dx, dx_act, dmid, dmid_act, din, din_act,
                                                              d_hidden, d_qkv, below_bias, acc, side, main)
                _, desc, evs_done, keep = ent
                _lib.check(k.lib.pm_vit_block_bwd(ctypes.byref(desc), _stream()), "pm_vit_block_bwd")
                pending[i] = evs_done
                if on_block_done is not None:
                    if len(evs_done) == 2:
                        last = k.side_stream2(main.device)
                        last.wait_event(evs_done[0])
                    else:
                        last = side
                    with torch.cuda.stream(last):
                        on_block_done(i)
                dx, dx_act = din, din_act
                continue
            if tr and not grouped:
                fork()
                with torch.cuda.stream(side):
                    k.linear_wgrad(dx_act, bw.h_act, gr["mlp.fc2.weight"], M, D, Hd, accumulate("mlp.fc2.weight", i))
            fuse_cs = tr and k.FUSE_COLSUM
            two = (grouped and k.GROUP_BIAS and not fuse_cs and
                   k.two_launch_group(M, ((D, Hd), (Hd, D), (D, D), (3 * D, D))))
            group_mlp = [(dx_act, bw.h_act, gr["mlp.fc2.weight"], accumulate("mlp.fc2.weight", i)),
                         (d_hidden, bw.ln2, gr["mlp.fc1.weight"], accumulate("mlp.fc1.weight", i),
                          gr["mlp.fc1.bias"] if (grouped and k.GROUP_BIAS and not fuse_cs) else None)] if grouped else None
            ev_mlp = None
            k.linear_dgrad(dx_act, p["mlp.fc2.weight"], d_hidden, M, D, Hd, EPI_DGELU, aux=bw.h_pre,
                           colsum=gr["mlp.fc1.bias"] if fuse_cs else None)
            if tr:
                fork()
                with torch.cuda.stream(side):
                    if not grouped:
                        k.linear_wgrad(d_hidden, bw.ln2, gr["mlp.fc1.weight"], M, Hd, D, accumulate("mlp.fc1.weight", i))
                    if not fuse_cs and not (grouped and k.GROUP_BIAS):
                        k.colsum(d_hidden, gr["mlp.fc1.bias"], M, Hd)
                    if two:
                        if not k.wgrad_group(group_mlp, M):
                            raise _lib.PolypMaeError("pm_wgrad_group refused a group that two_launch_group admitted")
                        ev_mlp = torch.cuda.Event()
                        ev_mlp.record(side)
            k.linear_dgrad(d_hidden, p["mlp.fc1.weight"], ws.d_ln, M, Hd, D)
            k.layernorm_bwd(ws.d_ln, bw.x_mid, p["norm2.weight"], bw.mean2, bw.rstd2, dx, dmid, dmid_act,
                            gr["norm2.weight"] if tr else None, gr["norm2.bias"] if tr else None,
                            gr["attn.proj.bias"] if tr else None, M, D)
            if tr and not grouped:
                fork()
                with torch.cuda.stream(side):
                    k.linear_wgrad(dmid_act, bw.attn, gr["attn.proj.weight"], M, D, D, accumulate("attn.proj.weight", i))
            k.linear_dgrad(dmid_act, p["attn.proj.weight"], ws.d_attn, M, D, D)
            k.attention_bwd(bw.qkv, bw.attn, ws.d_attn, bw.lse, ws.delta, d_qkv, B, N, g.heads, g.dh)
            if tr:
                last = k.side_stream2(main.device) if two else side
                ev = torch.cuda.Event()
                ev.record(main)
                last.wait_event(ev)
                with torch.cuda.stream(last):
                    gb = grouped and k.GROUP_BIAS
                    if not gb:
                        k.colsum(d_qkv, gr["attn.qkv.bias"], M, 3 * D)
                    if grouped:
                        group_attn = [(dmid_act, bw.attn, gr["attn.proj.weight"], accumulate("attn.proj.weight", i)),
                                      (d_qkv, bw.ln1, gr["attn.qkv.weight"], accumulate("attn.qkv.weight", i),
                                       gr["attn.qkv.bias"] if gb else None)]
                        ok = k.wgrad_group(group_attn, M, whole_k=True) if two else k.wgrad_group(group_mlp + group_attn, M)
                        if not ok:
                            raise _lib.PolypMaeError("pm_wgrad_group refused a group that can_group_wgrad admitted")
                    else:
                        k.linear_wgrad(d_qkv, bw.ln1, gr["attn.qkv.weight"], M, 3 * D, D, accumulate("attn.qkv.weight", i))
                    ev_last = torch.cuda.Event()
                    ev_last.record(last)
                    pending[i] = (ev_mlp, ev_last) if two else (ev_last,)
                    if on_block_done is not None:
                        if two:
                            last.wait_event(ev_mlp)
                        on_block_done(i)
            run_ln1 = need_dx_in or tr
            if run_ln1:
                k.linear_dgrad(d_qkv, p["attn.qkv.weight"], ws.d_ln, M, 3 * D, D)
            if not run_ln1:
                join(0)
                return None, None
            below_bias = None
            if i > 0 and trainable[i - 1]:
                below_bias = G[i - 1]["mlp.fc2.bias"]
            elif i == 0:
                below_bias = prev_bias_grad
            k.layernorm_bwd(ws.d_ln, xin, p["norm1.weight"], bw.mean1, bw.rstd1, dmid, din, din_act,
                            gr["norm1.weight"] if tr else None, gr["norm1.bias"] if tr else None, below_bias, M, D)
            dx, dx_act = din, din_act
            if on_block_done is not None and not tr:
                on_block_done(i)
        if defer_join:
            ws._deferred_join = [ev for j in sorted(pending, reverse=True) for ev in pending.pop(j)]
        else:
            join(0)
        return dx, dx_act

    def _top_block_sparse(self, ws, bw, p, gr, xin, dx, dx_act, sparse_top, last_bias_grad_done, dmid, din, din_act, d_qkv, below_bias,
                          acc, main, on_block_done, i, tr):
        k, g = self.k, self.g
        tc = self.top_compact(ws, g, k.act_dtype, dx.device)
        rows, inv = tc["rows"], tc["inv"]
        B, N, M, D, Hd = ws.B, ws.N, ws.M, g.dim, g.hidden
        R = B
        dev, f32 = dx.device, torch.float32
        e = lambda *s, dt=k.act_dtype: torch.empty(*s, dtype=dt, device=dev)
        dxc, dxac = dx.view(R, D), dx_act.view(R, D)
        G_ = (lambda n: gr[n]) if tr else (lambda n: None)
        if tr and not last_bias_grad_done:
            k.colsum(dxc, gr["mlp.fc2.bias"], R, D)
        d_hidden_c = e(R, Hd)
        k.linear_dgrad(dxac, p["mlp.fc2.weight"], d_hidden_c, R, D, Hd, EPI_DGELU, aux=tc["h_pre"])
        if tr:
            k.linear_wgrad(dxac, tc["h_act"], gr["mlp.fc2.weight"], R, D, Hd, acc("mlp.fc2.weight"), ws_name="_ws_front")
            k.linear_wgrad(d_hidden_c, tc["ln2"], gr["mlp.fc1.weight"], R, Hd, D, acc("mlp.fc1.weight"), ws_name="_ws_front")
            k.colsum(d_hidden_c, gr["mlp.fc1.bias"], R, Hd)
        d_ln_c = e(R, D)
        k.linear_dgrad(d_hidden_c, p["mlp.fc1.weight"], d_ln_c, R, Hd, D)
        dmid_c, dmid_act_c = e(R, D, dt=f32), e(R, D)
        k.layernorm_bwd(d_ln_c, tc["x_mid"], p["norm2.weight"], tc["mean2"], tc["rstd2"], dxc, dmid_c, dmid_act_c, G_("norm2.weight"),
                        G_("norm2.bias"), G_("attn.proj.bias"), R, D)
        if tr:
            k.linear_wgrad(dmid_act_c, tc["attn"], gr["attn.proj.weight"], R, D, D, acc("attn.proj.weight"), ws_name="_ws_front")
        d_attn_c = e(R, D)
        k.linear_dgrad(dmid_act_c, p["attn.proj.weight"], d_attn_c, R, D, D)
        k.scatter_rows_zero(dmid_c, inv, dmid.view(M, D))
        k.scatter_rows_zero(d_attn_c, inv, ws.d_attn.view(M, D))
        k.attention_bwd(bw.qkv, bw.attn, ws.d_attn, bw.lse, ws.delta, d_qkv, B, N, g.heads, g.dh)
        ev_last = None
        if tr:
            side = k.side_stream(main.device)
            ev = torch.cuda.Event()
            ev.record(main)
            side.wait_event(ev)
            with torch.cuda.stream(side):
                k.colsum(d_qkv, gr["attn.qkv.bias"], M, 3 * D)
                k.linear_wgrad(d_qkv, bw.ln1, gr["attn.qkv.weight"], M, 3 * D, D, acc("attn.qkv.weight"))
                ev_last = torch.cuda.Event()
                ev_last.record(side)
                if on_block_done is not None:
                    on_block_done(i)
        k.linear_dgrad(d_qkv, p["attn.qkv.weight"], ws.d_ln, M, 3 * D, D)
        k.layernorm_bwd(ws.d_ln, xin, p["norm1.weight"], bw.mean1, bw.rstd1, dmid, din, din_act, G_("norm1.weight"), G_("norm1.bias"),
                        below_bias, M, D)
        if not tr and on_block_done is not None:
            on_block_done(i)
        return (ev_last,) if ev_last is not None else None

    @staticmethod
    def join_deferred(ws: StackWorkspace) -> None:
        main = torch.cuda.current_stream()
        for ev in ws.__dict__.pop("_deferred_join", []):
            main.wait_event(ev)
```

ssl4polyp_amd/models.py:

```python
from __future__ import annotations

import math
from functools import partial
from typing import Dict, List, Optional

import numpy as np
import torch
import torch.nn as nn

from . import _lib
from .engine import (BLOCK_PARAM_NAMES, EPI_STORE, BlockStack, Kernels, StackGeom, StackWorkspace, _ptr, _stream)
from .flat import FlatParams

_DEFAULT_PRECISION = "bf16"


def get_1d_sincos_pos_embed_from_grid(embed_dim, pos):
    assert embed_dim % 2 == 0
    omega = np.arange(embed_dim // 2, dtype=np.float64)
    omega /= embed_dim / 2.0
    omega = 1.0 / 10000 ** omega
    out = np.einsum("m,d->md", pos.reshape(-1), omega)
    return np.concatenate([np.sin(out), np.cos(out)], axis=1)


def get_2d_sincos_pos_embed(embed_dim, grid_size, cls_token=False):
    grid_h = np.arange(grid_size, dtype=np.float32)
    grid_w = np.arange(grid_size, dtype=np.float32)
    grid = np.stack(np.meshgrid(grid_w, grid_h), axis=0).reshape([2, 1, grid_size, grid_size])
    assert embed_dim % 2 == 0
    emb = np.concatenate([get_1d_sincos_pos_embed_from_grid(embed_dim // 2, grid[0]),
                          get_1d_sincos_pos_embed_from_grid(embed_dim // 2, grid[1])], axis=1)
    if cls_token:
        emb = np.concatenate([np.zeros([1, embed_dim]), emb], axis=0)
    return emb


class PatchEmbed(nn.Module):
    def __init__(self, img_size=224, patch_size=16, in_chans=3, embed_dim=768):
        super().__init__()
        self.img_size = (img_size, img_size)
        self.patch_size = (patch_size, patch_size)
        self.grid_size = (img_size // patch_size, img_size // patch_size)
        self.num_patches = self.grid_size[0] * self.grid_size[1]
        self.proj = nn.Conv2d(in_chans, embed_dim, kernel_size=patch_size, stride=patch_size)


class Attention(nn.Module):
    def __init__(self, dim, num_heads, qkv_bias=True):
        super().__init__()
        self.num_heads = num_heads
        self.scale = (dim // num_heads) ** -0.5
        self.qkv = nn.Linear(dim, dim * 3, bias=qkv_bias)
        self.proj = nn.Linear(dim, dim)


class Mlp(nn.Module):
    def __init__(self, in_features, hidden_features):
        super().__init__()
        self.fc1 = nn.Linear(in_features, hidden_features)
        self.fc2 = nn.Linear(hidden_features, in_features)


class Block(nn.Module):
    def __init__(self, dim, num_heads, mlp_ratio=4.0, qkv_bias=True, norm_layer=nn.LayerNorm):
        super().__init__()
        self.norm1 = norm_layer(dim)
        self.attn = Attention(dim, num_heads, qkv_bias=qkv_bias)
        self.norm2 = norm_layer(dim)
        self.mlp = Mlp(dim, int(dim * mlp_ratio))


class _Runtime:

    def __init__(self, module: nn.Module, precision: str, enc: StackGeom, dec: Optional[StackGeom]):
        self.module = module
        self.precision = precision
        self.enc_geom, self.dec_geom = enc, dec
        self.k: Optional[Kernels] = None
        self.flat: Optional[FlatParams] = None
        self.pool: Dict[tuple, List[StackWorkspace]] = {}
        self.grad_sync = None
        self._wcache: Dict[str, tuple] = {}
        self.eps = 1e-6
        self.pending_updates: List[tuple] = []
        self.unused: tuple = ()

    def wait_updates(self, mat_through: Optional[int] = None, also=()) -> None:
        if not self.pending_updates:
            return
        last = -1
        for j, (r, lo, hi, ev) in enumerate(self.pending_updates):
            if mat_through is None or r == "vec" or lo < mat_through:
                last = j
        if last >= 0:
            ev = self.pending_updates[last][3]
            torch.cuda.current_stream().wait_event(ev)
            for st in also:
                st.wait_event(ev)
            del self.pending_updates[:last + 1]

    def block_end(self, prefix: str, i: int) -> int:
        f = self.flat
        j = f.index[f"{prefix}{i}.mlp.fc2.weight"]
        return f.offset[j] + f.numel[j]

    def ensure(self, device: torch.device) -> None:
        if device.type != "cuda":
            raise _lib.PolypMaeError("ssl4polyp_amd models run on the MI355X HIP path only (got a CPU tensor); "
                                     "there is no eager fallback")
        if self.k is None:
            self.k = Kernels(self.precision, self.eps)
        if self.flat is None or set(self.flat.names) != {n for n, _ in self.module.named_parameters()}:
            self.flat = FlatParams(self.module, self.k.act_dtype)
        if not self.flat.bound(device):
            self.flat.materialize(device)
            self.pool.clear()
            self._wcache = {}
        if self.flat.shadow_stale():
            self.wait_updates()
            self.k.cast(self.flat.P["mat"], self.flat.S)
            self.flat.mark_shadow_fresh()
        if self.pending_updates:
            f = self.flat
            self.wait_updates(mat_through=f.offset[f.index["blocks.0.attn.qkv.weight"]])

    def stack_weights(self, prefix: str, depth: int):
        hit = self._wcache.get(prefix)
        if hit is not None:
            return hit
        f = self.flat
        W, G = [], []
        for i in range(depth):
            w, g = {}, {}
            for n in BLOCK_PARAM_NAMES:
                full = f"{prefix}{i}.{n}"
                w[n] = f.shadow_view(full) if n.endswith("weight") and "norm" not in n else f.param_view(full)
                g[n] = f.grad_view(full)
            W.append(w)
            G.append(g)
        self._wcache[prefix] = (W, G)
        return W, G

    def get_ws(self, geom: StackGeom, B: int, N: int, training: bool) -> StackWorkspace:
        key = (geom.dim, geom.depth, B, N, training)
        lst = self.pool.setdefault(key, [])
        if lst:
            return lst.pop()
        return StackWorkspace(geom, B, N, self.k.act_dtype, self.flat.device, training)

    def put_ws(self, geom: StackGeom, ws: StackWorkspace) -> None:
        self.pool.setdefault((geom.dim, geom.depth, ws.B, ws.N, ws.training), []).append(ws)


def _update_gate(rt: _Runtime, prefix: str):
    if not rt.pending_updates:
        return None
    return lambda i, also=(): rt.wait_updates(mat_through=rt.block_end(prefix, i), also=also)


def _plan_grads(rt: _Runtime, names: List[str], needs: List[bool]):
    f = rt.flat
    tr = [n for n, need in zip(names, needs) if need and n not in rt.unused]
    flat_state = [f.grad_is_flat(n) for n in tr]
    if tr and all(flat_state):
        return True
    if any(flat_state):
        raise _lib.PolypMaeError("some parameter .grad tensors alias the engine's flat gradient buffer and others do "
                                 "not; call optimizer.zero_grad() for all parameters consistently")
    f.G["vec"].zero_()
    return False


class _EncoderFrontMixin:

    @staticmethod
    def front_fwd(rt: _Runtime, imgs, ids_keep, keep, pos_name="pos_embed"):
        k, f, mod = rt.k, rt.flat, rt.module
        B, C, img = imgs.shape[0], imgs.shape[1], imgs.shape[2]
        p = mod.patch_embed.patch_size[0]
        D = rt.enc_geom.dim
        PE = C * p * p
        PEp = k.padded_k(PE)
        dev = imgs.device
        cols = torch.empty(B * keep, PEp, dtype=k.act_dtype, device=dev)
        _lib.check(k.lib.pm_patch_im2col(_ptr(imgs), _ptr(ids_keep), _ptr(cols), PEp, k.act, B, C, img, p, keep, _stream()),
                   "pm_patch_im2col")
        emb = torch.empty(B * keep, D, dtype=torch.float32, device=dev)
        if PEp == PE:
            w = f.shadow_view("patch_embed.proj.weight").view(D, PE)
        else:
            w = k.pad_cast(f.param_view("patch_embed.proj.weight").view(D, PE), D, PEp)
        k.linear_fwd(cols, w, f.param_view("patch_embed.proj.bias"), emb, B * keep, D, PEp)
        x0 = torch.empty(B * (keep + 1), D, dtype=torch.float32, device=dev)
        _lib.check(k.lib.pm_assemble_tokens(_ptr(emb), _ptr(f.param_view("cls_token")), _ptr(f.param_view(pos_name)),
                                            _ptr(ids_keep), _ptr(x0), B, keep, D, _stream()), "pm_assemble_tokens")
        return cols, x0

    @staticmethod
    def front_bwd(rt: _Runtime, dx0, cols, ids_keep, B, keep, accumulate, need, learn_pos):
        k, f = rt.k, rt.flat
        D = rt.enc_geom.dim
        PEp = cols.shape[1]
        PE = f.param_view("patch_embed.proj.weight").numel() // D
        demb = torch.empty(B * keep, D, dtype=k.act_dtype, device=cols.device)
        dcls = f.grad_view("cls_token") if need("cls_token") else None
        dpos = f.grad_view("pos_embed") if learn_pos and need("pos_embed") else None
        if dpos is not None and ids_keep is None:
            _lib.check(k.lib.pm_assemble_tokens_bwd(_ptr(dx0), None, _ptr(demb), k.act, _ptr(dcls), None, B, keep, D,
                                                    _stream()), "pm_assemble_tokens_bwd")
            k.colsum(dx0.view(B, (keep + 1) * D), dpos.view(-1), B, (keep + 1) * D)
        else:
            _lib.check(k.lib.pm_assemble_tokens_bwd(_ptr(dx0), _ptr(ids_keep), _ptr(demb), k.act, _ptr(dcls), _ptr(dpos), B,
                                                    keep, D, _stream()), "pm_assemble_tokens_bwd")
        if need("patch_embed.proj.weight"):
            if PEp == PE:
                k.linear_wgrad(demb, cols, f.grad_view("patch_embed.proj.weight").view(D, PE), B * keep, D, PE, accumulate,
                               ws_name="_ws_front")
            else:
                dw = torch.empty(D, PEp, dtype=torch.float32, device=cols.device)
                k.linear_wgrad(demb, cols, dw, B * keep, D, PEp, False, ws_name="_ws_front")
                k.unpad_add(dw, f.grad_view("patch_embed.proj.weight").view(D, PE), accumulate)
        if need("patch_embed.proj.bias"):
            k.colsum(demb, f.grad_view("patch_embed.proj.bias"), B * keep, D)


class _VitClsFn(torch.autograd.Function):

    @staticmethod
    def forward(ctx, rt: _Runtime, imgs: torch.Tensor, pool: int, head: bool, names, *params):
        k, f, mod, g = rt.k, rt.flat, rt.module, rt.enc_geom
        B = imgs.shape[0]
        L = mod.patch_embed.num_patches
        N = L + 1
        D = g.dim
        needs = ctx.needs_input_grad[5:] if getattr(rt, "grad_enabled", True) else (False,) * len(params)
        below = any(nd for n, nd in zip(names, needs) if not n.startswith("lin_head"))
        training = any(needs)
        imgs = imgs.contiguous().float()
        cols, x0 = _EncoderFrontMixin.front_fwd(rt, imgs, None, L)
        ws = rt.get_ws(g, B, N, below)
        W, _ = rt.stack_weights("blocks.", g.depth)
        need_map = dict(zip(names, needs))
        front_needs = any(need_map.get(n, False) for n in ("cls_token", "pos_embed", "patch_embed.proj.weight", "patch_embed.proj.bias"))
        keep_from = 0 if front_needs else min((i for i in range(g.depth)
                                                if any(need_map.get(f"blocks.{i}.{n}", False) for n in BLOCK_PARAM_NAMES)), default=g.depth)
        cls_top = pool == 0 and k.SPARSE_TOP and N > 1 and (B % 8 == 0 or not any(needs))
        x = BlockStack(k, g).forward(ws, x0, W, before_block=_update_gate(rt, "blocks."), keep_from=keep_from, cls_top=cls_top)
        Nh = 1 if cls_top else N
        rt.wait_updates()
        dev = imgs.device
        f32 = torch.float32
        n_class = mod.lin_head.weight.shape[0] if head else 0
        feat = torch.empty(B, D, dtype=f32, device=dev)
        xhm = torch.empty(B, D, dtype=f32, device=dev) if pool else None
        mean = torch.empty(B * (N if pool else 1), dtype=f32, device=dev)
        rstd = torch.empty_like(mean)
        logits = torch.empty(B, n_class, dtype=f32, device=dev) if head else None
        _lib.check(k.lib.pm_vit_head_fwd(_ptr(x), Nh, pool, _ptr(f.param_view("norm.weight")), _ptr(f.param_view("norm.bias")),
                                         _ptr(f.param_view("lin_head.weight")) if head else None,
                                         _ptr(f.param_view("lin_head.bias")) if head else None, _ptr(feat), _ptr(xhm),
                                         _ptr(mean), _ptr(rstd), _ptr(logits), B, D, n_class, rt.eps, _stream()),
                   "pm_vit_head_fwd")
        if training:
            ctx.rt, ctx.names, ctx.ws = rt, names, ws
            if not below:
                x = x.clone() if pool else x.view(B, Nh, D)[:, 0].clone()
                rt.put_ws(g, ws)
                ctx.ws = None
                cols = x0 = None
            ctx.saved = (cols, x0, x, feat, xhm, mean, rstd)
            ctx.dims = (B, L, N, D, n_class, pool, head, below)
            ctx.cls_top = cls_top
        else:
            rt.put_ws(g, ws)
        return logits if head else feat

    @staticmethod
    def backward(ctx, dout):
        rt, names, ws = ctx.rt, ctx.names, ctx.ws
        k, f, mod, g = rt.k, rt.flat, rt.module, rt.enc_geom
        cols, x0, x, feat, xhm, mean, rstd = ctx.saved
        B, L, N, D, n_class, pool, head, below = ctx.dims
        needs = list(ctx.needs_input_grad[5:])
        need_map = dict(zip(names, needs))
        need = lambda n: need_map.get(n, False)
        accumulate = _plan_grads(rt, names, needs)
        if not accumulate and need("lin_head.weight"):
            f.grad_view("lin_head.weight").zero_()
        trainable = [any(need(f"blocks.{i}.{n}") for n in BLOCK_PARAM_NAMES) for i in range(g.depth)]
        learn_pos = need("pos_embed")
        front = need("cls_token") or need("patch_embed.proj.weight") or need("patch_embed.proj.bias") or \
            (learn_pos and need("pos_embed"))
        below_head = front or any(trainable)
        dout = dout.contiguous().float()
        cls_top = bool(getattr(ctx, "cls_top", False))
        if below_head and cls_top:
            tc = BlockStack.top_compact(ws, g, k.act_dtype, dout.device)
            dx, dx_act = tc["dx"], tc["dx_act"]
        else:
            dx = ws.dx[0] if below_head else None
            dx_act = ws.dx_act[0] if below_head else None
        x_rows = 1 if cls_top else (N if (below or pool) else 1)
        _lib.check(k.lib.pm_vit_head_bwd(
            _ptr(dout) if head else None, None if head else _ptr(dout), _ptr(x), x_rows, pool,
            _ptr(f.param_view("norm.weight")), _ptr(f.param_view("lin_head.weight")) if head else None, _ptr(feat), _ptr(xhm),
            _ptr(mean), _ptr(rstd), _ptr(dx), _ptr(dx_act), k.act,
            _ptr(f.grad_view("lin_head.weight")) if need("lin_head.weight") else None,
            _ptr(f.grad_view("lin_head.bias")) if need("lin_head.bias") else None,
            _ptr(f.grad_view("norm.weight")) if need("norm.weight") else None,
            _ptr(f.grad_view("norm.bias")) if need("norm.bias") else None, B, D, n_class, _stream()), "pm_vit_head_bwd")
        sync = rt.grad_sync
        if below_head:
            W, G = rt.stack_weights("blocks.", g.depth)
            cb = (lambda i: sync.block_done("blocks.", i)) if sync is not None else None
            dx0, _ = BlockStack(k, g).backward(ws, x0, W, G, dx, dx_act, False, trainable, front,
                                               lambda n, i: accumulate, cb, defer_join=k.DEFER_JOIN,
                                               sparse_top=True if cls_top else None)
            if front and dx0 is not None:
                _EncoderFrontMixin.front_bwd(rt, dx0, cols, None, B, L, accumulate, need, learn_pos)
            BlockStack.join_deferred(ws)
        if sync is not None:
            sync.backward_done()
        if ws is not None:
            rt.put_ws(g, ws)
        ctx.saved = None
        grads = [None if (accumulate or not nd or n in rt.unused) else f.grad_view(n) for n, nd in zip(names, needs)]
        return (None, None, None, None, None, *grads)


class _SupervisedLossFn(torch.autograd.Function):

    @staticmethod
    def forward(ctx, logits, targets, pos_weight, class_weights):
        if not logits.is_cuda:
            raise _lib.PolypMaeError("supervised_loss runs on the MI355X HIP path only (got a CPU tensor)")
        lib = _lib.load()
        logits = logits.contiguous().float()
        targets = targets.contiguous().to(torch.int64)
        B, C = logits.shape
        loss = torch.empty(1, dtype=torch.float32, device=logits.device)
        dlogits = torch.empty_like(logits)
        _lib.check(lib.pm_supervised_loss_fwd(_ptr(logits), _ptr(targets), _ptr(pos_weight), _ptr(class_weights), _ptr(loss),
                                              _ptr(dlogits), B, C, _stream()), "pm_supervised_loss_fwd")
        ctx.dlogits = dlogits
        return loss.reshape(())

    @staticmethod
    def backward(ctx, dloss):
        lib = _lib.load()
        d = ctx.dlogits
        out = torch.empty_like(d)
        dloss = dloss.reshape(1).contiguous().float()
        _lib.check(lib.pm_scale(_ptr(d), _ptr(dloss), _ptr(out), d.numel(), _stream()), "pm_scale")
        return out, None, None, None


def supervised_loss(logits: torch.Tensor, targets: torch.Tensor, pos_weight=None, class_weights=None) -> torch.Tensor:
    dev = logits.device
    if pos_weight is not None and not torch.is_tensor(pos_weight):
        pos_weight = torch.tensor(float(pos_weight), dtype=torch.float32, device=dev)
    if pos_weight is not None:
        pos_weight = pos_weight.to(device=dev, dtype=torch.float32).reshape(1)
    if class_weights is not None:
        class_weights = class_weights.to(device=dev, dtype=torch.float32).contiguous()
        if class_weights.numel() != logits.shape[1]:
            raise ValueError("class_weights must have one entry per class")
    if logits.ndim != 2 or logits.shape[1] < 2:
        raise ValueError("supervised_loss expects logits [B, n_class >= 2]")
    if not logits.is_cuda:
        raise _lib.PolypMaeError("supervised_loss runs on the MI355X HIP path only (got a CPU tensor)")
    from . import ops
    return torch.ops.polypmae.supervised_loss(logits, targets, pos_weight, class_weights)


class _MaeFn(torch.autograd.Function):

    @staticmethod
    def forward(ctx, rt: _Runtime, imgs, noise, mask_ratio, names, *params):
        k, f, mod, ge, gd = rt.k, rt.flat, rt.module, rt.enc_geom, rt.dec_geom
        B, C, img = imgs.shape[0], imgs.shape[1], imgs.shape[2]
        p = mod.patch_embed.patch_size[0]
        L = mod.patch_embed.num_patches
        keep = int(L * (1 - mask_ratio))
        if keep < 1:
            raise ValueError("mask_ratio leaves no visible patch")
        De, Dd, PE = ge.dim, gd.dim, p * p * C
        dev = imgs.device
        f32 = torch.float32
        training = any(ctx.needs_input_grad) and getattr(rt, "grad_enabled", True)
        imgs = imgs.contiguous().float()
        ctx.set_materialize_grads(False)
        ids_shuffle = torch.empty(B, L, dtype=torch.int32, device=dev)
        ids_restore = torch.empty(B, L, dtype=torch.int32, device=dev)
        mask = torch.empty(B, L, dtype=f32, device=dev)
        noise = noise.contiguous().float()
        _lib.check(k.lib.pm_mae_masking(_ptr(noise), _ptr(ids_shuffle), _ptr(ids_restore), _ptr(mask), B, L, keep,
                                        _stream()), "pm_mae_masking")
        ids_keep = ids_shuffle[:, :keep].contiguous()
        cols, x0 = _EncoderFrontMixin.front_fwd(rt, imgs, ids_keep, keep)
        ws_e = rt.get_ws(ge, B, keep + 1, training)
        We, _ = rt.stack_weights("blocks.", ge.depth)
        xe = BlockStack(k, ge).forward(ws_e, x0, We, before_block=_update_gate(rt, "blocks."))
        rt.wait_updates()
        Me, Md = B * (keep + 1), B * (L + 1)
        latent = torch.empty(Me, De, dtype=k.act_dtype, device=dev)
        mean_e, rstd_e = torch.empty(Me, dtype=f32, device=dev), torch.empty(Me, dtype=f32, device=dev)
        k.layernorm_fwd(xe, f.param_view("norm.weight"), f.param_view("norm.bias"), latent, mean_e, rstd_e, Me, De)
        demb = torch.empty(Me, Dd, dtype=f32, device=dev)
        k.linear_fwd(latent, f.shadow_view("decoder_embed.weight"), f.param_view("decoder_embed.bias"), demb, Me, Dd, De)
        xd0 = torch.empty(Md, Dd, dtype=f32, device=dev)
        _lib.check(k.lib.pm_mae_unshuffle(_ptr(demb), _ptr(f.param_view("mask_token")),
                                          _ptr(f.param_view("decoder_pos_embed")), _ptr(ids_restore), _ptr(xd0), B, L,
                                          keep, Dd, _stream()), "pm_mae_unshuffle")
        ws_d = rt.get_ws(gd, B, L + 1, training)
        Wd, _ = rt.stack_weights("decoder_blocks.", gd.depth)
        xd = BlockStack(k, gd).forward(ws_d, xd0, Wd)
        yn = torch.empty(Md, Dd, dtype=k.act_dtype, device=dev)
        mean_d, rstd_d = torch.empty(Md, dtype=f32, device=dev), torch.empty(Md, dtype=f32, device=dev)
        k.layernorm_fwd(xd, f.param_view("decoder_norm.weight"), f.param_view("decoder_norm.bias"), yn, mean_d, rstd_d,
                        Md, Dd)
        pred_full = torch.empty(B, L + 1, PE, dtype=f32, device=dev)
        k.linear_fwd(yn, f.shadow_view("decoder_pred.weight"), f.param_view("decoder_pred.bias"), pred_full, Md, PE, Dd)
        patch_loss = torch.empty(B * L, dtype=f32, device=dev)
        sums = torch.empty(2, dtype=f32, device=dev)
        loss = torch.empty(1, dtype=f32, device=dev)
        npx = 1 if mod.norm_pix_loss else 0
        _lib.check(k.lib.pm_mae_loss_fwd(_ptr(imgs), _ptr(pred_full), PE, 1, _ptr(patch_loss), B, C, img, p, npx,
                                         _stream()), "pm_mae_loss_fwd")
        _lib.check(k.lib.pm_mae_loss_finish(_ptr(patch_loss), _ptr(mask), B * L, _ptr(sums), _ptr(loss), _stream()),
                   "pm_mae_loss_finish")
        pred = pred_full[:, 1:, :]
        if training:
            ctx.rt, ctx.names = rt, names
            ctx.ws = (ws_e, ws_d)
            ctx.saved = (imgs, ids_keep, ids_shuffle, mask, cols, x0, xe, latent, mean_e, rstd_e, xd0, xd, yn, mean_d,
                         rstd_d, pred_full, sums)
            ctx.dims = (B, C, img, p, L, keep, npx)
            ctx.mark_non_differentiable(mask)
        else:
            rt.put_ws(ge, ws_e)
            rt.put_ws(gd, ws_d)
        return loss.reshape(()), pred, mask

    @staticmethod
    def backward(ctx, dloss, dpred, dmask):
        if dpred is not None:
            raise NotImplementedError("gradients flowing into `pred` from outside the MAE loss are not supported")
        rt, names = ctx.rt, ctx.names
        k, f, mod, ge, gd = rt.k, rt.flat, rt.module, rt.enc_geom, rt.dec_geom
        ws_e, ws_d = ctx.ws
        (imgs, ids_keep, ids_shuffle, mask, cols, x0, xe, latent, mean_e, rstd_e, xd0, xd, yn, mean_d, rstd_d, pred_full,
         sums) = ctx.saved
        B, C, img, p, L, keep, npx = ctx.dims
        De, Dd, PE = ge.dim, gd.dim, p * p * C
        Me, Md = B * (keep + 1), B * (L + 1)
        dev = imgs.device
        needs = list(ctx.needs_input_grad[5:])
        need_map = dict(zip(names, needs))
        need = lambda n: need_map.get(n, False)
        accumulate = _plan_grads(rt, names, needs)
        acc_fn = lambda n, i: accumulate
        sync = rt.grad_sync
        if dloss is None:
            dloss = torch.zeros((), dtype=torch.float32, device=dev)
        dloss = dloss.reshape(1).contiguous().float()
        PEp = k.padded_k(PE)
        dpred_act = torch.empty(Md, PEp, dtype=k.act_dtype, device=dev)
        _lib.check(k.lib.pm_mae_loss_bwd(_ptr(imgs), _ptr(pred_full), PE, 1, _ptr(mask), _ptr(sums), _ptr(dloss),
                                         _ptr(dpred_act), PEp, k.act, B, C, img, p, npx, _stream()), "pm_mae_loss_bwd")
        if PEp == PE:
            if need("decoder_pred.weight"):
                k.linear_wgrad(dpred_act, yn, f.grad_view("decoder_pred.weight"), Md, PE, Dd, accumulate)
            if need("decoder_pred.bias"):
                k.colsum(dpred_act, f.grad_view("decoder_pred.bias"), Md, PE)
            k.linear_dgrad(dpred_act, f.shadow_view("decoder_pred.weight"), ws_d.d_ln, Md, PE, Dd)
        else:
            if need("decoder_pred.weight"):
                dw = torch.empty(PEp, Dd, dtype=torch.float32, device=dev)
                k.linear_wgrad(dpred_act, yn, dw, Md, PEp, Dd, False)
                k.unpad_add(dw, f.grad_view("decoder_pred.weight").view(PE, Dd), accumulate)
            if need("decoder_pred.bias"):
                db = torch.zeros(1, PEp, dtype=torch.float32, device=dev)
                k.colsum(dpred_act, db, Md, PEp)
                k.unpad_add(db, f.grad_view("decoder_pred.bias").view(1, PE), True)
            wpad = k.pad_cast(f.param_view("decoder_pred.weight").view(PE, Dd), PEp, Dd)
            k.linear_dgrad(dpred_act, wpad, ws_d.d_ln, Md, PEp, Dd)
        Wd, Gd = rt.stack_weights("decoder_blocks.", gd.depth)
        tr_d = [any(need(f"decoder_blocks.{i}.{n}") for n in BLOCK_PARAM_NAMES) for i in range(gd.depth)]
        last = gd.depth - 1
        k.layernorm_bwd(ws_d.d_ln, xd, f.param_view("decoder_norm.weight"), mean_d, rstd_d, None, ws_d.dx[last & 1 ^ 1],
                        ws_d.dx_act[last & 1 ^ 1],
                        f.grad_view("decoder_norm.weight") if need("decoder_norm.weight") else None,
                        f.grad_view("decoder_norm.bias") if need("decoder_norm.bias") else None,
                        Gd[last]["mlp.fc2.bias"] if tr_d[last] else None, Md, Dd)
        cb_d = (lambda i: sync.block_done("decoder_blocks.", i)) if sync is not None else None
        dxd0, _ = BlockStack(k, gd).backward(ws_d, xd0, Wd, Gd, ws_d.dx[last & 1 ^ 1], ws_d.dx_act[last & 1 ^ 1], True, tr_d,
                                             True, acc_fn, cb_d, ends_pass=False)
        demb_act = torch.empty(Me, Dd, dtype=k.act_dtype, device=dev)
        cs_ws = k._scratch("_ws_cs_main", k._need(("unshuf", Dd), lambda: k.lib.pm_workspace_bytes(_lib.WS_UNSHUFFLE_BWD, 1, Dd)), dev)
        _lib.check(k.lib.pm_mae_unshuffle_bwd(_ptr(dxd0), _ptr(ids_shuffle), _ptr(demb_act), k.act,
                                              _ptr(f.grad_view("mask_token")) if need("mask_token") else None, B, L, keep,
                                              Dd, _ptr(cs_ws), cs_ws.numel(), _stream()), "pm_mae_unshuffle_bwd")
        if need("decoder_embed.weight"):
            k.linear_wgrad(demb_act, latent, f.grad_view("decoder_embed.weight"), Me, Dd, De, accumulate)
        if need("decoder_embed.bias"):
            k.colsum(demb_act, f.grad_view("decoder_embed.bias"), Me, Dd)
        k.linear_dgrad(demb_act, f.shadow_view("decoder_embed.weight"), ws_e.d_ln, Me, Dd, De)
        We, Ge = rt.stack_weights("blocks.", ge.depth)
        tr_e = [any(need(f"blocks.{i}.{n}") for n in BLOCK_PARAM_NAMES) for i in range(ge.depth)]
        last = ge.depth - 1
        k.layernorm_bwd(ws_e.d_ln, xe, f.param_view("norm.weight"), mean_e, rstd_e, None, ws_e.dx[last & 1 ^ 1],
                        ws_e.dx_act[last & 1 ^ 1], f.grad_view("norm.weight") if need("norm.weight") else None,
                        f.grad_view("norm.bias") if need("norm.bias") else None,
                        Ge[last]["mlp.fc2.bias"] if tr_e[last] else None, Me, De)
        front = need("cls_token") or need("patch_embed.proj.weight") or need("patch_embed.proj.bias")
        cb_e = (lambda i: sync.block_done("blocks.", i)) if sync is not None else None
        dx0, _ = BlockStack(k, ge).backward(ws_e, x0, We, Ge, ws_e.dx[last & 1 ^ 1], ws_e.dx_act[last & 1 ^ 1], True, tr_e,
                                            front, acc_fn, cb_e, defer_join=k.DEFER_JOIN)
        if front and dx0 is not None:
            _EncoderFrontMixin.front_bwd(rt, dx0, cols, ids_keep, B, keep, accumulate, need, False)
        BlockStack.join_deferred(ws_e)
        if sync is not None:
            sync.backward_done()
        rt.put_ws(ge, ws_e)
        rt.put_ws(gd, ws_d)
        ctx.saved = None
        grads = [None if (accumulate or not nd) else f.grad_view(n) for n, nd in zip(names, needs)]
        return (None, None, None, None, None, *grads)


class MaskedAutoencoderViT(nn.Module):

    def state_dict(self, *args, **kwargs):
        self._rt.wait_updates()
        return super().state_dict(*args, **kwargs)

    def __init__(self, img_size=224, patch_size=16, in_chans=3, embed_dim=1024, depth=24, num_heads=16,
                 decoder_embed_dim=512, decoder_depth=8, decoder_num_heads=16, mlp_ratio=4.0, norm_layer=nn.LayerNorm,
                 norm_pix_loss=False, precision: Optional[str] = None):
        super().__init__()
        eps = self._check_norm(norm_layer)
        self.patch_embed = PatchEmbed(img_size, patch_size, in_chans, embed_dim)
        num_patches = self.patch_embed.num_patches
        self.cls_token = nn.Parameter(torch.zeros(1, 1, embed_dim))
        self.pos_embed = nn.Parameter(torch.zeros(1, num_patches + 1, embed_dim), requires_grad=False)
        self.blocks = nn.ModuleList([Block(embed_dim, num_heads, mlp_ratio, qkv_bias=True, norm_layer=norm_layer)
                                     for _ in range(depth)])
        self.norm = norm_layer(embed_dim)
        self.decoder_embed = nn.Linear(embed_dim, decoder_embed_dim, bias=True)
        self.mask_token = nn.Parameter(torch.zeros(1, 1, decoder_embed_dim))
        self.decoder_pos_embed = nn.Parameter(torch.zeros(1, num_patches + 1, decoder_embed_dim), requires_grad=False)
        self.decoder_blocks = nn.ModuleList([
            Block(decoder_embed_dim, decoder_num_heads, mlp_ratio, qkv_bias=True, norm_layer=norm_layer)
            for _ in range(decoder_depth)])
        self.decoder_norm = norm_layer(decoder_embed_dim)
        self.decoder_pred = nn.Linear(decoder_embed_dim, patch_size ** 2 * in_chans, bias=True)
        self.norm_pix_loss = norm_pix_loss
        self.initialize_weights()
        enc = StackGeom(embed_dim, num_heads, depth, int(embed_dim * mlp_ratio))
        dec = StackGeom(decoder_embed_dim, decoder_num_heads, decoder_depth, int(decoder_embed_dim * mlp_ratio))
        object.__setattr__(self, "_rt", _Runtime(self, precision or _DEFAULT_PRECISION, enc, dec))
        self._rt.eps = eps

    @staticmethod
    def _check_norm(norm_layer):
        probe = norm_layer(8)
        if not isinstance(probe, nn.LayerNorm) or not probe.elementwise_affine:
            raise ValueError("only affine nn.LayerNorm is supported by the HIP path")
        return float(probe.eps)

    def initialize_weights(self):
        gs = int(self.patch_embed.num_patches ** 0.5)
        pos_embed = get_2d_sincos_pos_embed(self.pos_embed.shape[-1], gs, cls_token=True)
        self.pos_embed.data.copy_(torch.from_numpy(pos_embed).float().unsqueeze(0))
        dpos = get_2d_sincos_pos_embed(self.decoder_pos_embed.shape[-1], gs, cls_token=True)
        self.decoder_pos_embed.data.copy_(torch.from_numpy(dpos).float().unsqueeze(0))
        w = self.patch_embed.proj.weight.data
        torch.nn.init.xavier_uniform_(w.view([w.shape[0], -1]))
        torch.nn.init.normal_(self.cls_token, std=0.02)
        torch.nn.init.normal_(self.mask_token, std=0.02)
        self.apply(self._init_weights)

    def _init_weights(self, m):
        if isinstance(m, nn.Linear):
            torch.nn.init.xavier_uniform_(m.weight)
            if m.bias is not None:
                nn.init.constant_(m.bias, 0)
        elif isinstance(m, nn.LayerNorm):
            nn.init.constant_(m.bias, 0)
            nn.init.constant_(m.weight, 1.0)

    def patchify(self, imgs):
        p = self.patch_embed.patch_size[0]
        n, c, hh, ww = imgs.shape
        if hh != ww or hh % p or c != 3:
            raise ValueError(f"patchify expects square 3-channel images whose side is a multiple of {p} (got {tuple(imgs.shape)})")
        g = hh // p
        return imgs.view(n, c, g, p, g, p).permute(0, 2, 4, 3, 5, 1).reshape(n, g * g, p * p * c)

    def unpatchify(self, x):
        p = self.patch_embed.patch_size[0]
        n, L, _ = x.shape
        g = math.isqrt(L)
        if g * g != L:
            raise ValueError(f"unpatchify expects a square number of patches (got {L})")
        return x.view(n, g, g, p, p, 3).permute(0, 5, 1, 3, 2, 4).reshape(n, 3, g * p, g * p)

    def _draw_noise(self, B: int, device) -> torch.Tensor:
        if torch.cuda.is_current_stream_capturing():
            raise _lib.PolypMaeError("MAE forward under stream capture: the masking draw would be baked into the graph (the same "
                                     "masks at every replay) -- pass `noise=` from a buffer the caller refills between replays")
        L = self.patch_embed.num_patches
        n = B * L
        gen = torch.cuda.default_generators[device.index if device.index is not None else torch.cuda.current_device()]
        seed = int(gen.initial_seed()) & 0xFFFFFFFFFFFFFFFF
        off = int(gen.get_offset())
        gen.set_offset(off + 4 * ((n + 3) // 4))
        key = (seed ^ ((off >> 32) * 0x9E3779B97F4A7C15)) & 0xFFFFFFFFFFFFFFFF
        noise = torch.empty(B, L, dtype=torch.float32, device=device)
        _lib.check(self._rt.k.lib.pm_mae_noise(_ptr(noise), n, key, off & 0xFFFFFFFF, _stream()), "pm_mae_noise")
        return noise

    def forward(self, imgs, mask_ratio=0.75, noise: Optional[torch.Tensor] = None):
        rt = self._rt
        rt.ensure(imgs.device)
        assert imgs.shape[2] == self.patch_embed.img_size[0] and imgs.shape[3] == self.patch_embed.img_size[1]
        if noise is None:
            noise = self._draw_noise(imgs.shape[0], imgs.device)
        from . import ops
        return torch.ops.polypmae.mae_forward(imgs, noise, float(mask_ratio), ops.register_runtime(rt), list(rt.flat.params))


def mae_vit_base_patch16_dec512d8b(**kwargs):
    return MaskedAutoencoderViT(patch_size=16, embed_dim=768, depth=12, num_heads=12, decoder_embed_dim=512,
                                decoder_depth=8, decoder_num_heads=16, mlp_ratio=4,
                                norm_layer=partial(nn.LayerNorm, eps=1e-6), **kwargs)


def mae_vit_large_patch16_dec512d8b(**kwargs):
    return MaskedAutoencoderViT(patch_size=16, embed_dim=1024, depth=24, num_heads=16, decoder_embed_dim=512,
                                decoder_depth=8, decoder_num_heads=16, mlp_ratio=4,
                                norm_layer=partial(nn.LayerNorm, eps=1e-6), **kwargs)


def mae_vit_huge_patch14_dec512d8b(**kwargs):
    return MaskedAutoencoderViT(patch_size=14, embed_dim=1280, depth=32, num_heads=16, decoder_embed_dim=512,
                                decoder_depth=8, decoder_num_heads=16, mlp_ratio=4,
                                norm_layer=partial(nn.LayerNorm, eps=1e-6), **kwargs)


mae_vit_base_patch16 = mae_vit_base_patch16_dec512d8b
mae_vit_large_patch16 = mae_vit_large_patch16_dec512d8b
mae_vit_huge_patch14 = mae_vit_huge_patch14_dec512d8b


class _ClassifierBase(nn.Module):
    def state_dict(self, *args, **kwargs):
        self._rt.wait_updates()
        return super().state_dict(*args, **kwargs)

    def _classify(self, imgs):
        if self.dense:
            raise NotImplementedError("dense (DPT decoder) mode is dead code on the reference's path (every caller "
                                      "passes dense=None, tc.py:5646-5654) and is not built")
        if self.out_token not in ("cls", "spatial"):
            raise ValueError(f"out_token must be 'cls' or 'spatial' (got {self.out_token!r})")
        head = bool(self.head if isinstance(self.head, bool) else self.head_bool)
        rt = self._rt
        rt.ensure(imgs.device)
        assert imgs.shape[2] == self.patch_embed.img_size[0] and imgs.shape[3] == self.patch_embed.img_size[1]
        from . import ops
        return torch.ops.polypmae.vit_forward(imgs, ops.register_runtime(rt), 1 if self.out_token == "spatial" else 0, head,
                                              list(rt.flat.params))


class ViT_from_MAE(_ClassifierBase):

    def __init__(self, weight_path, head, num_classes, frozen, dense, embed_dim, depth, num_heads, out_token,
                 precision: Optional[str] = None):
        super().__init__()
        norm_layer = partial(nn.LayerNorm, eps=1e-6)
        full = MaskedAutoencoderViT(patch_size=16, embed_dim=embed_dim, depth=depth, num_heads=num_heads,
                                    decoder_embed_dim=512, decoder_depth=8, decoder_num_heads=16, mlp_ratio=4,
                                    norm_layer=norm_layer)
        if weight_path is not None:
            weights = torch.load(weight_path, map_location="cpu", weights_only=False)["model"]
            own = full.state_dict()
            n = 0
            for name, param in weights.items():
                if name in own:
                    own[name].copy_(param)
                    n += 1
            print(f"Successfully loaded params for {n} items")
        self.patch_embed = full.patch_embed
        self.cls_token = full.cls_token
        self.pos_embed = full.pos_embed
        self.blocks = full.blocks
        self.norm = full.norm
        self.decoder_pos_embed = full.decoder_pos_embed
        self.norm_pix_loss = False
        self.head = head
        if head:
            self.lin_head = nn.Linear(embed_dim, num_classes)
        self.frozen = frozen
        self.dense = dense
        self.out_token = out_token
        self._learned_pos = False
        enc = StackGeom(embed_dim, num_heads, depth, int(embed_dim * 4))
        object.__setattr__(self, "_rt", _Runtime(self, precision or _DEFAULT_PRECISION, enc, None))
        self._rt.unused = ("decoder_pos_embed",)

    def load_my_state_dict(self, state_dict):
        own_state = self.state_dict()
        i = 0
        for name, param in state_dict.items():
            if name not in own_state:
                continue
            own_state[name].copy_(param)
            i += 1
        print(f"Successfully loaded params for {i} items")

    def forward(self, imgs):
        return self._classify(imgs)


class VisionTransformer_from_Any(_ClassifierBase):

    def __init__(self, head, num_classes, frozen, dense, embed_dim, depth, num_heads, out_token, ImageNet_weights=False,
                 precision: Optional[str] = None):
        super().__init__()
        norm_layer = partial(nn.LayerNorm, eps=1e-6)
        self.num_features = self.embed_dim = embed_dim
        self.patch_embed = PatchEmbed(224, 16, 3, embed_dim)
        self.cls_token = nn.Parameter(torch.zeros(1, 1, embed_dim))
        self.pos_embed = nn.Parameter(torch.zeros(1, self.patch_embed.num_patches + 1, embed_dim))
        self.pos_drop = nn.Dropout(p=0.0)
        self.blocks = nn.Sequential(*[Block(embed_dim, num_heads, 4.0, qkv_bias=True, norm_layer=norm_layer)
                                      for _ in range(depth)])
        self.norm = norm_layer(embed_dim)
        self.pre_logits = nn.Identity()
        _timm_head = nn.Linear(embed_dim, 1000)
        nn.init.trunc_normal_(self.pos_embed, std=0.02)
        nn.init.trunc_normal_(self.cls_token, std=0.02)
        nn.init.zeros_(_timm_head.weight)
        for m in self.modules():
            if isinstance(m, nn.Linear):
                nn.init.trunc_normal_(m.weight, std=0.02)
                nn.init.zeros_(m.bias)
            elif isinstance(m, nn.LayerNorm):
                nn.init.zeros_(m.bias)
                nn.init.ones_(m.weight)
        if ImageNet_weights:
            import os
            loc = ImageNet_weights if isinstance(ImageNet_weights, (str, os.PathLike)) else os.environ.get("SSL4POLYP_AUGREG_NPZ")
            if not loc or not os.path.exists(str(loc)):
                raise FileNotFoundError("ImageNet_weights=True needs the augreg ViT-B/16 .npz of models.py:51-55 on local disk: "
                                        "pass its path as ImageNet_weights or set SSL4POLYP_AUGREG_NPZ (no download here)")
            self.load_pretrained(loc)
        self.head = nn.Identity()
        self.head_bool = head
        if head:
            self.lin_head = nn.Linear(embed_dim, num_classes)
        self.frozen = frozen
        self.dense = dense
        self.out_token = out_token
        self._learned_pos = True
        enc = StackGeom(embed_dim, num_heads, depth, int(embed_dim * 4))
        object.__setattr__(self, "_rt", _Runtime(self, precision or _DEFAULT_PRECISION, enc, None))

    def load_pretrained(self, checkpoint_path):
        if str(checkpoint_path).lower().endswith(".npz"):
            return load_augreg_npz(self, str(checkpoint_path))
        checkpoint = torch.load(str(checkpoint_path), map_location="cpu", weights_only=False)
        state_dict = None
        if isinstance(checkpoint, dict):
            for key in ("state_dict", "model", "model_state", "weights", "params"):
                if isinstance(checkpoint.get(key), dict):
                    state_dict = checkpoint[key]
                    break
            if state_dict is None and all(isinstance(k, str) for k in checkpoint.keys()):
                state_dict = checkpoint
        if not isinstance(state_dict, dict):
            print(f"Warning: unsupported checkpoint format for {checkpoint_path!s}: {type(checkpoint)}")
            return
        missing, unexpected = self.load_state_dict(state_dict, strict=False)
        if missing:
            print(f"Missing keys when loading pretrained weights: {missing}")
        if unexpected:
            print(f"Unexpected keys when loading pretrained weights: {unexpected}")

    def forward(self, x):
        return self._classify(x)


def load_augreg_npz(model, path: str, prefix: str = "") -> None:
    w = np.load(path)
    if not prefix and "opt/target/embedding/kernel" in w:
        prefix = "opt/target/"

    def t(a):
        if a.ndim == 4:
            a = a.transpose(3, 2, 0, 1)
        elif a.ndim == 3:
            a = a.transpose(2, 0, 1)
        elif a.ndim == 2:
            a = a.transpose(1, 0)
        return torch.from_numpy(np.ascontiguousarray(a))

    def raw(a):
        return torch.from_numpy(np.ascontiguousarray(a))

    with torch.no_grad():
        ew = t(w[f"{prefix}embedding/kernel"])
        if ew.shape != model.patch_embed.proj.weight.shape:
            raise ValueError(f"patch embedding {tuple(ew.shape)} does not fit {tuple(model.patch_embed.proj.weight.shape)}")
        model.patch_embed.proj.weight.copy_(ew)
        model.patch_embed.proj.bias.copy_(raw(w[f"{prefix}embedding/bias"]))
        model.cls_token.copy_(raw(w[f"{prefix}cls"]).reshape(model.cls_token.shape))
        pos = raw(w[f"{prefix}Transformer/posembed_input/pos_embedding"])
        if pos.shape != model.pos_embed.shape:
            raise ValueError(f"pos_embedding {tuple(pos.shape)} != {tuple(model.pos_embed.shape)} (bicubic resize of the "
                             "table is not on this path: the reference runs at 224^2 / patch 16)")
        model.pos_embed.copy_(pos)
        model.norm.weight.copy_(raw(w[f"{prefix}Transformer/encoder_norm/scale"]))
        model.norm.bias.copy_(raw(w[f"{prefix}Transformer/encoder_norm/bias"]))
        for i, blk in enumerate(model.blocks.children()):
            bp = f"{prefix}Transformer/encoderblock_{i}/"
            mp = bp + "MultiHeadDotProductAttention_1/"
            blk.norm1.weight.copy_(raw(w[bp + "LayerNorm_0/scale"]))
            blk.norm1.bias.copy_(raw(w[bp + "LayerNorm_0/bias"]))
            blk.attn.qkv.weight.copy_(torch.cat([raw(w[f"{mp}{n}/kernel"]).flatten(1).T for n in ("query", "key", "value")]))
            blk.attn.qkv.bias.copy_(torch.cat([raw(w[f"{mp}{n}/bias"]).reshape(-1) for n in ("query", "key", "value")]))
            blk.attn.proj.weight.copy_(t(w[mp + "out/kernel"]).flatten(1))
            blk.attn.proj.bias.copy_(raw(w[mp + "out/bias"]))
            for r in range(2):
                fc = getattr(blk.mlp, f"fc{r + 1}")
                fc.weight.copy_(t(w[f"{bp}MlpBlock_3/Dense_{r}/kernel"]))
                fc.bias.copy_(raw(w[f"{bp}MlpBlock_3/Dense_{r}/bias"]))
            blk.norm2.weight.copy_(raw(w[bp + "LayerNorm_2/scale"]))
            blk.norm2.bias.copy_(raw(w[bp + "LayerNorm_2/bias"]))


def get_MAE_backbone(weight_path, head, num_classes, frozen, dense, out_token="cls", precision=None):
    return ViT_from_MAE(weight_path, head, num_classes, frozen, dense, embed_dim=768, depth=12, num_heads=12,
                        out_token=out_token, precision=precision)


def get_ImageNet_or_random_ViT(head, num_classes, frozen, dense, ImageNet_weights, out_token="cls", precision=None):
    return VisionTransformer_from_Any(head, num_classes, frozen, dense, 768, 12, 12, out_token, ImageNet_weights,
                                      precision=precision)
```

Baseline: 6343 images/sec.

## Move LayerNorm param-grad reductions and top-block weight grads to side stream

LayerNorm backward is split into a partials kernel on the main stream and a batched reduce kernel. The reduce handles both block LayerNorms in one launch and runs on a side stream after an event, so it no longer blocks the dgrad critical path. For the sparse CLS-top block, the head's parameter grads, MLP/proj weight grads and the LN reduce are also deferred to the side stream. This is meant to overlap them with the main-stream dgrad chain. It costs per-block partial workspaces, double-buffered top-block scratch and more event synchronization.

```diff
diff --git a/include/polypmae.h b/include/polypmae.h
--- a/include/polypmae.h
+++ b/include/polypmae.h
@@ -28,6 +28,16 @@
                      const float* rstd, const float* dres, long lddres, float* dx, long lddx, void* dx_act,
                      int act_dtype, float* dgamma, float* dbeta, float* dcolsum, int M, int D, void* workspace,
                      size_t ws_bytes, void* stream);
+
+typedef struct pm_ln_reduce_item {
+  const float* partials;
+  int nblocks, D;
+  float *dgamma, *dbeta, *dcolsum;
+} pm_ln_reduce_item;
+int pm_layernorm_bwd_partials(const void* dy, int dy_dtype, const float* x, long ldx, const float* gamma, const float* mean,
+                              const float* rstd, const float* dres, long lddres, float* dx, long lddx, void* dx_act,
+                              int act_dtype, int M, int D, void* workspace, size_t ws_bytes, int* nblocks, void* stream);
+int pm_layernorm_bwd_reduce(const pm_ln_reduce_item* items, int n, void* stream);
 
 int pm_gemm(const void* A, long lda, int a_kmajor, const void* B, long ldb, int b_kmajor, int in_dtype,
             const float* bias, void* C, long ldc, int c_dtype, int epilogue, void* aux, const float* resid,
@@ -226,6 +236,13 @@
 } pm_block_bwd_desc;
 int pm_vit_block_bwd(const pm_block_bwd_desc* d, void* stream);
 
+typedef struct pm_block_bwd_side {
+  void *ws_ln2, *ws_ln1;
+  size_t ws_ln_bytes;
+  void *ev_ln, *ev_side_done;
+} pm_block_bwd_side;
+int pm_vit_block_bwd_side(const pm_block_bwd_desc* d, const pm_block_bwd_side* s, void* stream);
+
 int pm_vit_head_fwd(const float* x, int N, int pool, const float* gamma, const float* beta, const float* W,
                     const float* bias, float* feat, float* xhat_mean, float* mean, float* rstd, float* logits, int B, int D,
                     int n_class, float eps, void* stream);
diff --git a/ssl4polyp_amd/_lib.py b/ssl4polyp_amd/_lib.py
--- a/ssl4polyp_amd/_lib.py
+++ b/ssl4polyp_amd/_lib.py
@@ -15,8 +15,11 @@
 SIGNATURES = {
     "pm_layernorm_fwd": [P, L, P, P, P, I, P, P, I, I, F, P],
     "pm_layernorm_bwd": [P, I, P, L, P, P, P, P, L, P, L, P, I, P, P, P, I, I, P, ctypes.c_size_t, P],
+    "pm_layernorm_bwd_partials": [P, I, P, L, P, P, P, P, L, P, L, P, I, I, I, P, ctypes.c_size_t, P, P],
+    "pm_layernorm_bwd_reduce": [P, I, P],
     "pm_vit_block_fwd": [P, P],
     "pm_vit_block_bwd": [P, P],
+    "pm_vit_block_bwd_side": [P, P, P],
     "pm_gemm": [P, L, I, P, L, I, I, P, P, L, I, I, P, P, I, I, I, P],
     "pm_gemm_ws": [P, L, I, P, L, I, I, P, P, L, I, I, P, P, I, I, I, P, ctypes.c_size_t, P],
     "pm_gemm_ex": [P, L, I, P, L, I, I, P, P, L, I, I, P, P, I, I, I, P, ctypes.c_size_t, P, P],
@@ -107,6 +110,16 @@
                 [(n, c_void_p) for n in ("side_stream2", "ev_fork2", "ev_done2")])
 
 
+class BlockBwdSide(ctypes.Structure):
+    _fields_ = [("ws_ln2", c_void_p), ("ws_ln1", c_void_p), ("ws_ln_bytes", ctypes.c_size_t), ("ev_ln", c_void_p),
+                ("ev_side_done", c_void_p)]
+
+
+class LnReduceItem(ctypes.Structure):
+    _fields_ = [("partials", c_void_p), ("nblocks", c_int), ("D", c_int), ("dgamma", c_void_p), ("dbeta", c_void_p),
+                ("dcolsum", c_void_p)]
+
+
 class BlockFwdDesc(ctypes.Structure):
     _fields_ = ([(n, c_void_p) for n in ("x", "x_mid", "x_out", "ln1", "mean1", "rstd1", "qkv", "lse", "attn", "ln2", "mean2",
                                         "rstd2", "h_pre", "h_act", "norm1_w", "norm1_b", "norm2_w", "norm2_b", "qkv_w", "proj_w",
diff --git a/ssl4polyp_amd/csrc/pm_block.hip b/ssl4polyp_amd/csrc/pm_block.hip
--- a/ssl4polyp_amd/csrc/pm_block.hip
+++ b/ssl4polyp_amd/csrc/pm_block.hip
@@ -27,8 +27,9 @@
                     Hd, nullptr, 0, &opts, stream);
 }
 
-extern "C" int pm_vit_block_bwd(const pm_block_bwd_desc* d, void* stream) {
+static int block_bwd(const pm_block_bwd_desc* d, const pm_block_bwd_side* s, void* stream) {
   if (!d) return PM_EINVAL;
+  if (s && (!s->ws_ln2 || !s->ws_ln1 || s->ws_ln2 == s->ws_ln1 || !s->ev_ln || !s->ev_side_done)) return PM_EINVAL;
   if (!d->x_in || !d->x_mid || !d->ln1 || !d->qkv || !d->attn || !d->ln2 || !d->h_pre || !d->h_act || !d->dx || !d->dx_act ||
       !d->dmid || !d->dmid_act || !d->din || !d->din_act || !d->d_hidden || !d->d_qkv || !d->d_ln || !d->d_attn || !d->delta)
     return PM_EINVAL;
@@ -36,6 +37,7 @@
   if (d->samples <= 0 || d->N <= 0 || d->D <= 0 || d->Hd <= 0 || d->heads <= 0 || (d->D % d->heads)) return PM_ESHAPE;
   if (d->dtype != PM_BF16 && d->dtype != PM_F16 && d->dtype != PM_F32) return PM_EINVAL;
   const int M = d->samples * d->N, D = d->D, Hd = d->Hd, dt = d->dtype;
+  if (s && s->ws_ln_bytes < pm_workspace_bytes(PM_WS_LAYERNORM_BWD, M, D)) return PM_EINVAL;
   hipStream_t main = pm_stream(stream), side = pm_stream(d->side_stream);
   pm_gemm_opts opts;
   opts.max_blocks = 0;
@@ -79,9 +81,17 @@
   if ((st = pm_gemm_ex(d->d_hidden, Hd, 0, d->fc1_w, D, 1, dt, nullptr, d->d_ln, D, dt, PM_EPI_STORE, nullptr, nullptr, M, D, Hd,
                        nullptr, 0, &opts, stream)))
     return st;
-  if ((st = pm_layernorm_bwd(d->d_ln, dt, d->x_mid, D, d->norm2_w, d->mean2, d->rstd2, d->dx, D, d->dmid, D, d->dmid_act, dt,
-                             d->g_norm2_w, d->g_norm2_b, d->g_proj_b, M, D, d->ws_ln, d->ws_ln_bytes, stream)))
+  pm_ln_reduce_item red[2];
+  if (s) {
+    int nb = 0;
+    if ((st = pm_layernorm_bwd_partials(d->d_ln, dt, d->x_mid, D, d->norm2_w, d->mean2, d->rstd2, d->dx, D, d->dmid, D, d->dmid_act,
+                                        dt, M, D, s->ws_ln2, s->ws_ln_bytes, &nb, stream)))
+      return st;
+    red[0] = pm_ln_reduce_item{(const float*)s->ws_ln2, nb, D, d->g_norm2_w, d->g_norm2_b, d->g_proj_b};
+  } else if ((st = pm_layernorm_bwd(d->d_ln, dt, d->x_mid, D, d->norm2_w, d->mean2, d->rstd2, d->dx, D, d->dmid, D, d->dmid_act, dt,
+                                    d->g_norm2_w, d->g_norm2_b, d->g_proj_b, M, D, d->ws_ln, d->ws_ln_bytes, stream))) {
     return st;
+  }
   if ((st = pm_gemm_ex(d->dmid_act, D, 0, d->proj_w, D, 1, dt, nullptr, d->d_attn, D, dt, PM_EPI_STORE, nullptr, nullptr, M, D, D,
                        nullptr, 0, &opts, stream)))
     return st;
@@ -102,6 +112,25 @@
   if ((st = pm_gemm_ex(d->d_qkv, 3 * D, 0, d->qkv_w, D, 1, dt, nullptr, d->d_ln, D, dt, PM_EPI_STORE, nullptr, nullptr, M, D, 3 * D,
                        nullptr, 0, &opts, stream)))
     return st;
-  return pm_layernorm_bwd(d->d_ln, dt, d->x_in, D, d->norm1_w, d->mean1, d->rstd1, d->dmid, D, d->din, D, d->din_act, dt,
-                          d->g_norm1_w, d->g_norm1_b, d->g_below_bias, M, D, d->ws_ln, d->ws_ln_bytes, stream);
+  if (!s)
+    return pm_layernorm_bwd(d->d_ln, dt, d->x_in, D, d->norm1_w, d->mean1, d->rstd1, d->dmid, D, d->din, D, d->din_act, dt,
+                            d->g_norm1_w, d->g_norm1_b, d->g_below_bias, M, D, d->ws_ln, d->ws_ln_bytes, stream);
+  int nb = 0;
+  if ((st = pm_layernorm_bwd_partials(d->d_ln, dt, d->x_in, D, d->norm1_w, d->mean1, d->rstd1, d->dmid, D, d->din, D, d->din_act, dt,
+                                      M, D, s->ws_ln1, s->ws_ln_bytes, &nb, stream)))
+    return st;
+  red[1] = pm_ln_reduce_item{(const float*)s->ws_ln1, nb, D, d->g_norm1_w, d->g_norm1_b, d->g_below_bias};
+  hipStream_t last = two ? side2 : side;
+  if (hipEventRecord((hipEvent_t)s->ev_ln, main) != hipSuccess) return PM_ELAUNCH;
+  if (hipStreamWaitEvent(last, (hipEvent_t)s->ev_ln, 0) != hipSuccess) return PM_ELAUNCH;
+  if ((st = pm_layernorm_bwd_reduce(red, 2, two ? d->side_stream2 : d->side_stream))) return st;
+  if (hipEventRecord((hipEvent_t)s->ev_side_done, last) != hipSuccess) return PM_ELAUNCH;
+  return PM_OK;
 }
+
+extern "C" int pm_vit_block_bwd(const pm_block_bwd_desc* d, void* stream) { return block_bwd(d, nullptr, stream); }
+
+extern "C" int pm_vit_block_bwd_side(const pm_block_bwd_desc* d, const pm_block_bwd_side* s, void* stream) {
+  if (!s) return PM_EINVAL;
+  return block_bwd(d, s, stream);
+}
diff --git a/ssl4polyp_amd/csrc/pm_layernorm.hip b/ssl4polyp_amd/csrc/pm_layernorm.hip
--- a/ssl4polyp_amd/csrc/pm_layernorm.hip
+++ b/ssl4polyp_amd/csrc/pm_layernorm.hip
@@ -187,16 +187,21 @@
   }
 }
 
-__global__ __launch_bounds__(1024) void ln_bwd_reduce_kernel(const float* __restrict__ partials, float* dgamma, float* dbeta,
-                                                             float* dcolsum, int nblocks, int D) {
+struct ln_reduce_args {
+  pm_ln_reduce_item it[4];
+};
+
+__global__ __launch_bounds__(1024) void ln_bwd_reduce_kernel(ln_reduce_args a) {
   __shared__ float red[16][64];
+  const pm_ln_reduce_item& it = a.it[blockIdx.z];
+  const int D = it.D;
   const int lane = threadIdx.x & 63, rg = threadIdx.x >> 6;
   const int d = blockIdx.x * 64 + lane;
   const int v = blockIdx.y;
-  float* dst = v == 0 ? dgamma : (v == 1 ? dbeta : dcolsum);
+  float* dst = v == 0 ? it.dgamma : (v == 1 ? it.dbeta : it.dcolsum);
   if (!dst) return;
   float s0 = 0.f;
-  if (d < D) s0 = strided_sum<16>(partials + (long)v * D + d, 3L * D, rg, 16, nblocks);
+  if (d < D) s0 = strided_sum<16>(it.partials + (long)v * D + d, 3L * D, rg, 16, it.nblocks);
   red[rg][lane] = s0;
   __syncthreads();
   if (rg == 0 && d < D) {
@@ -228,13 +233,72 @@
   return pm_check_launch();
 }
 
+namespace {
+
+int ln_bwd_launch(const void* dy, int dy_dtype, const float* x, long ldx, const float* gamma, const float* mean, const float* rstd,
+                   const float* dres, long lddres, float* dx, long lddx, void* dx_act, float* dgamma, float* dbeta, float* dcolsum,
+                   float* partials, int M, int D, int grid, hipStream_t s) {
+  const int nv = (D + 255) / 256;
+#define PM_LN_BWD(TD, NV)                                                                                               \
+  hipLaunchKernelGGL((ln_bwd_kernel<TD, TD, NV>), dim3(grid), dim3(256), 0, s, (const TD*)dy, x, ldx, gamma, mean, rstd, \
+                     dres, lddres, dx, lddx, (TD*)dx_act, dgamma, dbeta, dcolsum, partials, M, D)
+  PM_DISPATCH_ACT(dy_dtype, T, {
+    if (nv == 1) PM_LN_BWD(T, 1); else if (nv == 2) PM_LN_BWD(T, 2); else if (nv == 3) PM_LN_BWD(T, 3);
+    else if (nv == 4) PM_LN_BWD(T, 4); else PM_LN_BWD(T, 5);
+  });
+#undef PM_LN_BWD
+  return PM_OK;
+}
+
+int ln_bwd_check(const void* dy, int dy_dtype, const float* x, long ldx, const float* gamma, const float* mean, const float* rstd,
+                 const float* dres, long lddres, float* dx, long lddx, void* dx_act, int act_dtype, int M, int D) {
+  if (!dy || !x || !gamma || !mean || !rstd || !dx) return PM_EINVAL;
+  if (M <= 0 || D <= 0 || D > kMaxD || (D & 3) || (ldx & 3) || (lddx & 3) || (dres && (lddres & 3))) return PM_ESHAPE;
+  if (dx_act && act_dtype != dy_dtype) return PM_EINVAL;
+  return PM_OK;
+}
+
+}
+
+extern "C" int pm_layernorm_bwd_reduce(const pm_ln_reduce_item* items, int n, void* stream) {
+  if (!items || n < 1 || n > 4) return PM_EINVAL;
+  ln_reduce_args a;
+  int maxD = 0;
+  for (int j = 0; j < n; ++j) {
+    if (!items[j].partials) return PM_EINVAL;
+    if (items[j].nblocks <= 0 || items[j].nblocks > 1024 || items[j].D <= 0 || items[j].D > kMaxD || (items[j].D & 3)) return PM_ESHAPE;
+    a.it[j] = items[j];
+    if (items[j].D > maxD) maxD = items[j].D;
+  }
+  for (int j = n; j < 4; ++j) a.it[j] = pm_ln_reduce_item{nullptr, 0, 0, nullptr, nullptr, nullptr};
+  hipLaunchKernelGGL(ln_bwd_reduce_kernel, dim3((maxD + 63) / 64, 3, n), dim3(1024), 0, pm_stream(stream), a);
+  return pm_check_launch();
+}
+
+extern "C" int pm_layernorm_bwd_partials(const void* dy, int dy_dtype, const float* x, long ldx, const float* gamma,
+                                         const float* mean, const float* rstd, const float* dres, long lddres, float* dx,
+                                         long lddx, void* dx_act, int act_dtype, int M, int D, void* workspace, size_t ws_bytes,
+                                         int* nblocks, void* stream) {
+  if (!nblocks) return PM_EINVAL;
+  if (int st = ln_bwd_check(dy, dy_dtype, x, ldx, gamma, mean, rstd, dres, lddres, dx, lddx, dx_act, act_dtype, M, D)) return st;
+  if (!workspace || ws_bytes < pm_workspace_bytes(PM_WS_LAYERNORM_BWD, M, D)) return PM_EINVAL;
+  int grid = (M + 3) / 4;
+  int cap = (int)(ws_bytes / ((size_t)3 * D * sizeof(float)));
+  if (cap > 1024) cap = 1024;
+  if (grid > cap) grid = cap;
+  float* partials = reinterpret_cast<float*>(workspace);
+  if (int st = ln_bwd_launch(dy, dy_dtype, x, ldx, gamma, mean, rstd, dres, lddres, dx, lddx, dx_act, partials, partials, partials,
+                             partials, M, D, grid, pm_stream(stream)))
+    return st;
+  *nblocks = grid;
+  return pm_check_launch();
+}
+
 extern "C" int pm_layernorm_bwd(const void* dy, int dy_dtype, const float* x, long ldx, const float* gamma,
                                 const float* mean, const float* rstd, const float* dres, long lddres, float* dx,
                                 long lddx, void* dx_act, int act_dtype, float* dgamma, float* dbeta, float* dcolsum,
                                 int M, int D, void* workspace, size_t ws_bytes, void* stream) {
-  if (!dy || !x || !gamma || !mean || !rstd || !dx) return PM_EINVAL;
-  if (M <= 0 || D <= 0 || D > kMaxD || (D & 3) || (ldx & 3) || (lddx & 3) || (dres && (lddres & 3))) return PM_ESHAPE;
-  if (dx_act && act_dtype != dy_dtype) return PM_EINVAL;
+  if (int st = ln_bwd_check(dy, dy_dtype, x, ldx, gamma, mean, rstd, dres, lddres, dx, lddx, dx_act, act_dtype, M, D)) return st;
   int grid = (M + 3) / 4;
   float* partials = nullptr;
   const bool want_sums = dgamma || dbeta || dcolsum;
@@ -248,16 +312,12 @@
   }
   if (grid < 1) grid = 1;
   hipStream_t s = pm_stream(stream);
-  const int nv = (D + 255) / 256;
-#define PM_LN_BWD(TD, NV)                                                                                               \
-  hipLaunchKernelGGL((ln_bwd_kernel<TD, TD, NV>), dim3(grid), dim3(256), 0, s, (const TD*)dy, x, ldx, gamma, mean, rstd, \
-                     dres, lddres, dx, lddx, (TD*)dx_act, dgamma, dbeta, dcolsum, partials, M, D)
-  PM_DISPATCH_ACT(dy_dtype, T, {
-    if (nv == 1) PM_LN_BWD(T, 1); else if (nv == 2) PM_LN_BWD(T, 2); else if (nv == 3) PM_LN_BWD(T, 3);
-    else if (nv == 4) PM_LN_BWD(T, 4); else PM_LN_BWD(T, 5);
-  });
-#undef PM_LN_BWD
-  if (partials)
-    hipLaunchKernelGGL(ln_bwd_reduce_kernel, dim3((D + 63) / 64, 3), dim3(1024), 0, s, partials, dgamma, dbeta, dcolsum, grid, D);
+  if (int st = ln_bwd_launch(dy, dy_dtype, x, ldx, gamma, mean, rstd, dres, lddres, dx, lddx, dx_act, dgamma, dbeta, dcolsum, partials,
+                             M, D, grid, s))
+    return st;
+  if (partials) {
+    const pm_ln_reduce_item it = {partials, grid, D, dgamma, dbeta, dcolsum};
+    return pm_layernorm_bwd_reduce(&it, 1, stream);
+  }
   return pm_check_launch();
 }
diff --git a/ssl4polyp_amd/engine.py b/ssl4polyp_amd/engine.py
--- a/ssl4polyp_amd/engine.py
+++ b/ssl4polyp_amd/engine.py
@@ -79,6 +79,25 @@
                                              _ptr(rstd), _ptr(dres), D, _ptr(dx), D, _ptr(dx_act), self.act,
                                              _ptr(dgamma), _ptr(dbeta), _ptr(dcolsum), M, D, _ptr(ws), ws.numel(), _stream()),
                    "pm_layernorm_bwd")
+
+    def layernorm_bwd_partials(self, dy, x, gamma, mean, rstd, dres, dx, dx_act, M, D, ws) -> int:
+        nb = ctypes.c_int(0)
+        _lib.check(self.lib.pm_layernorm_bwd_partials(_ptr(dy), _lib.dtype_code(dy.dtype), _ptr(x), D, _ptr(gamma), _ptr(mean),
+                                                      _ptr(rstd), _ptr(dres), D, _ptr(dx), D, _ptr(dx_act), self.act, M, D,
+                                                      _ptr(ws), ws.numel(), ctypes.byref(nb), _stream()), "pm_layernorm_bwd_partials")
+        return nb.value
+
+    def layernorm_bwd_reduce(self, items):
+        arr = (_lib.LnReduceItem * len(items))(*[_lib.LnReduceItem(_ptr(w), nb, D, _ptr(a), _ptr(b), _ptr(c))
+                                                 for w, nb, D, a, b, c in items])
+        _lib.check(self.lib.pm_layernorm_bwd_reduce(arr, len(items), _stream()), "pm_layernorm_bwd_reduce")
+
+    def ln_partials_buffer(self, M: int, D: int, device) -> torch.Tensor:
+        return torch.empty(self._need(("ln", M, D), lambda: self.lib.pm_workspace_bytes(_lib.WS_LAYERNORM_BWD, M, D)),
+                           dtype=torch.uint8, device=device)
+
+    LN_REDUCE_SIDE = os.environ.get("PM_LN_REDUCE_SIDE", "1") != "0"
+    TOP_SIDE = os.environ.get("PM_TOP_SIDE", "1") != "0"
 
     SPLIT_FORWARD = int(os.environ.get("PM_SPLIT_FWD", "2"))
     WGRAD_BLOCKS = int(os.environ.get("PM_WGRAD_BLOCKS", "128"))
@@ -417,7 +436,9 @@
             inv[rows.long()] = torch.arange(B, dtype=torch.int32, device=dev)
             tc = ws.__dict__["_top_c"] = dict(
                 rows=rows, inv=inv, x=e(B, D, dt=f32), attn=e(B, D), x_mid=e(B, D, dt=f32), ln2=e(B, D), mean2=e(B, dt=f32),
-                rstd2=e(B, dt=f32), h_pre=e(B, Hd), h_act=e(B, Hd), x_out=e(B, D, dt=f32), dx=e(B, D, dt=f32), dx_act=e(B, D))
+                rstd2=e(B, dt=f32), h_pre=e(B, Hd), h_act=e(B, Hd), x_out=e(B, D, dt=f32), dx=e(B, D, dt=f32), dx_act=e(B, D),
+                bwd=[dict(d_hidden=e(B, Hd), d_ln=e(B, D), dmid=e(B, D, dt=f32), dmid_act=e(B, D), d_attn=e(B, D), ws_ln=None)
+                     for _ in range(2)], turn=0)
         return tc
 
     def _top_block_forward_cls(self, ws, bw, p, x, parts, main, keep: bool) -> torch.Tensor:
@@ -461,7 +482,8 @@
             v(p["attn.qkv.bias"]), v(p["attn.proj.bias"]), v(p["mlp.fc1.bias"]), v(p["mlp.fc2.bias"]),
             (b1 - b0) * N, b1 - b0, N, D, Hd, g.heads, k.act, k.gemm_variant, k.eps)
 
-    def _bwd_desc(self, ws, bw, p, gr, xin, dx, dx_act, dmid, dmid_act, din, din_act, d_hidden, d_qkv, below_bias, acc, side, main):
+    def _bwd_desc(self, ws, bw, p, gr, xin, dx, dx_act, dmid, dmid_act, din, din_act, d_hidden, d_qkv, below_bias, acc, side, main,
+                  parity: int = 0):
         k, g = self.k, self.g
         M, D, Hd = ws.M, g.dim, g.hidden
         v = lambda t: t.data_ptr() if t is not None else None
@@ -494,14 +516,26 @@
             side.cuda_stream, None, ev_fork.cuda_event, ev_done.cuda_event,
             ws.B, ws.N, D, Hd, g.heads, k.act, k.gemm_variant, k.GROUP_BLOCKS_SLICED if need else k.GROUP_BLOCKS, acc,
             int(two), side2.cuda_stream if two else None, ev_fork2.cuda_event if two else None, ev_done2.cuda_event if two else None)
-        return desc, (ev_done, ev_done2) if two else (ev_done,), (ev_fork, ev_fork2, ws_ln, ws_group)
+        keep = (ev_fork, ev_fork2, ws_ln, ws_group)
+        if k.LN_REDUCE_SIDE:
+            bufs = ws.__dict__.setdefault("_ln_partials", {})
+            if parity not in bufs:
+                bufs[parity] = (k.ln_partials_buffer(M, D, dx.device), k.ln_partials_buffer(M, D, dx.device))
+            p2, p1 = bufs[parity]
+            ev_ln, ev_side_done = torch.cuda.Event(), torch.cuda.Event()
+            ev_ln.record(main)
+            ev_side_done.record(main)
+            sd = _lib.BlockBwdSide(v(p2), v(p1), p2.numel(), ev_ln.cuda_event, ev_side_done.cuda_event)
+            keep += (sd, ev_ln, ev_side_done, p2, p1)
+        return desc, (ev_done, ev_done2) if two else (ev_done,), keep
 
     def backward(self, ws: StackWorkspace, x_in: torch.Tensor, W, G, dx: torch.Tensor, dx_act: torch.Tensor,
                  last_bias_grad_done: bool, trainable: Sequence[bool], need_input_grad: bool,
                  accumulate: Callable[[str, int], bool], on_block_done: Optional[Callable[[int], None]] = None,
                  prev_bias_grad: Optional[torch.Tensor] = None,
                  ends_pass: bool = True, defer_join: bool = False,
-                 sparse_top: Optional[Tuple[torch.Tensor, torch.Tensor]] = None) -> Tuple[Optional[torch.Tensor], Optional[torch.Tensor]]:
+                 sparse_top: Optional[Tuple[torch.Tensor, torch.Tensor]] = None,
+                 top_side_work: Optional[Callable[[], None]] = None) -> Tuple[Optional[torch.Tensor], Optional[torch.Tensor]]:
         k, g = self.k, self.g
         B, N, M, D, Hd = ws.B, ws.N, ws.M, g.dim, g.hidden
         lowest = min([i for i, t in enumerate(trainable) if t], default=g.depth)
@@ -535,7 +569,7 @@
                     raise _lib.PolypMaeError("the cls-row top block needs a batch that is a multiple of 8 to train (16-byte k-major rows)")
                 below_bias = (G[i - 1]["mlp.fc2.bias"] if trainable[i - 1] else None) if i > 0 else prev_bias_grad
                 ev_last = self._top_block_sparse(ws, bw, p, gr, xin, dx, dx_act, sparse_top, last_bias_grad_done, dmid, din, din_act,
-                                                 d_qkv, below_bias, lambda n: accumulate(n, i), main, on_block_done, i, tr)
+                                                 d_qkv, below_bias, lambda n: accumulate(n, i), main, on_block_done, i, tr, top_side_work)
                 if ev_last is not None:
                     pending[i] = ev_last
                 dx, dx_act = din, din_act
@@ -556,15 +590,19 @@
                        int(accumulate("mlp.fc1.weight", i)) << 2 | int(accumulate("mlp.fc2.weight", i)) << 3)
                 key = (dx.data_ptr(), dx_act.data_ptr(), xin.data_ptr(), gr["attn.qkv.weight"].data_ptr(),
                        p["attn.qkv.weight"].data_ptr(), gr["norm1.weight"].data_ptr(),
-                       below_bias.data_ptr() if below_bias is not None else 0, acc, k.gemm_variant, k.GROUP_BLOCKS, k.GROUP_BLOCKS_SLICED, k.TWO_GROUPS, k.TIME_BLOCK_EVENTS,
+                       below_bias.data_ptr() if below_bias is not None else 0, acc, k.gemm_variant, k.GROUP_BLOCKS, k.GROUP_BLOCKS_SLICED, k.TWO_GROUPS, k.LN_REDUCE_SIDE, k.TIME_BLOCK_EVENTS,
                        ptr_of(k.__dict__.get("_ws_ln")), ptr_of(k.__dict__.get("_ws_group")))
                 ent = bcache.get(i)
                 if ent is None or ent[0] != key:
                     ent = bcache[i] = (key,) + self._bwd_desc(ws, bw, p, gr, xin, dx, dx_act, dmid, dmid_act, din, din_act,
-                                                              d_hidden, d_qkv, below_bias, acc, side, main)
+                                                              d_hidden, d_qkv, below_bias, acc, side, main, parity=o)
                 _, desc, evs_done, keep = ent
-                _lib.check(k.lib.pm_vit_block_bwd(ctypes.byref(desc), _stream()), "pm_vit_block_bwd")
-                pending[i] = evs_done
+                if len(keep) > 4:
+                    _lib.check(k.lib.pm_vit_block_bwd_side(ctypes.byref(desc), ctypes.byref(keep[4]), _stream()), "pm_vit_block_bwd_side")
+                    pending[i] = evs_done[:-1] + (keep[6],)
+                else:
+                    _lib.check(k.lib.pm_vit_block_bwd(ctypes.byref(desc), _stream()), "pm_vit_block_bwd")
+                    pending[i] = evs_done
                 if on_block_done is not None:
                     if len(evs_done) == 2:
                         last = k.side_stream2(main.device)
@@ -658,52 +696,86 @@
         return dx, dx_act
 
     def _top_block_sparse(self, ws, bw, p, gr, xin, dx, dx_act, sparse_top, last_bias_grad_done, dmid, din, din_act, d_qkv, below_bias,
-                          acc, main, on_block_done, i, tr):
+                          acc, main, on_block_done, i, tr, side_work=None):
         k, g = self.k, self.g
         tc = self.top_compact(ws, g, k.act_dtype, dx.device)
         rows, inv = tc["rows"], tc["inv"]
         B, N, M, D, Hd = ws.B, ws.N, ws.M, g.dim, g.hidden
         R = B
-        dev, f32 = dx.device, torch.float32
-        e = lambda *s, dt=k.act_dtype: torch.empty(*s, dtype=dt, device=dev)
         dxc, dxac = dx.view(R, D), dx_act.view(R, D)
         G_ = (lambda n: gr[n]) if tr else (lambda n: None)
-        if tr and not last_bias_grad_done:
+        tb = tc["bwd"][tc["turn"]]
+        tc["turn"] ^= 1
+        side = k.side_stream(main.device) if tr else None
+        top_side = tr and k.TOP_SIDE and not torch.cuda.is_current_stream_capturing()
+        wsn = "_ws" if top_side else "_ws_front"
+
+        if side_work is not None and not top_side:
+            side_work()
+        if tr and not last_bias_grad_done and not top_side:
             k.colsum(dxc, gr["mlp.fc2.bias"], R, D)
-        d_hidden_c = e(R, Hd)
+        d_hidden_c = tb["d_hidden"]
         k.linear_dgrad(dxac, p["mlp.fc2.weight"], d_hidden_c, R, D, Hd, EPI_DGELU, aux=tc["h_pre"])
-        if tr:
-            k.linear_wgrad(dxac, tc["h_act"], gr["mlp.fc2.weight"], R, D, Hd, acc("mlp.fc2.weight"), ws_name="_ws_front")
-            k.linear_wgrad(d_hidden_c, tc["ln2"], gr["mlp.fc1.weight"], R, Hd, D, acc("mlp.fc1.weight"), ws_name="_ws_front")
+
+        def mlp_grads():
+            k.linear_wgrad(dxac, tc["h_act"], gr["mlp.fc2.weight"], R, D, Hd, acc("mlp.fc2.weight"), ws_name=wsn)
+            k.linear_wgrad(d_hidden_c, tc["ln2"], gr["mlp.fc1.weight"], R, Hd, D, acc("mlp.fc1.weight"), ws_name=wsn)
             k.colsum(d_hidden_c, gr["mlp.fc1.bias"], R, Hd)
-        d_ln_c = e(R, D)
+
+        if tr and not top_side:
+            mlp_grads()
+        d_ln_c = tb["d_ln"]
         k.linear_dgrad(d_hidden_c, p["mlp.fc1.weight"], d_ln_c, R, Hd, D)
-        dmid_c, dmid_act_c = e(R, D, dt=f32), e(R, D)
-        k.layernorm_bwd(d_ln_c, tc["x_mid"], p["norm2.weight"], tc["mean2"], tc["rstd2"], dxc, dmid_c, dmid_act_c, G_("norm2.weight"),
-                        G_("norm2.bias"), G_("attn.proj.bias"), R, D)
-        if tr:
-            k.linear_wgrad(dmid_act_c, tc["attn"], gr["attn.proj.weight"], R, D, D, acc("attn.proj.weight"), ws_name="_ws_front")
-        d_attn_c = e(R, D)
+        dmid_c, dmid_act_c = tb["dmid"], tb["dmid_act"]
+        nb = 0
+        if top_side:
+            if tb["ws_ln"] is None:
+                tb["ws_ln"] = k.ln_partials_buffer(R, D, dx.device)
+            nb = k.layernorm_bwd_partials(d_ln_c, tc["x_mid"], p["norm2.weight"], tc["mean2"], tc["rstd2"], dxc, dmid_c, dmid_act_c,
+                                          R, D, tb["ws_ln"])
+        else:
+            k.layernorm_bwd(d_ln_c, tc["x_mid"], p["norm2.weight"], tc["mean2"], tc["rstd2"], dxc, dmid_c, dmid_act_c,
+                            G_("norm2.weight"), G_("norm2.bias"), G_("attn.proj.bias"), R, D)
+        proj_grad = lambda: k.linear_wgrad(dmid_act_c, tc["attn"], gr["attn.proj.weight"], R, D, D, acc("attn.proj.weight"), ws_name=wsn)
+        if tr and not top_side:
+            proj_grad()
+        d_attn_c = tb["d_attn"]
         k.linear_dgrad(dmid_act_c, p["attn.proj.weight"], d_attn_c, R, D, D)
         k.scatter_rows_zero(dmid_c, inv, dmid.view(M, D))
         k.scatter_rows_zero(d_attn_c, inv, ws.d_attn.view(M, D))
         k.attention_bwd(bw.qkv, bw.attn, ws.d_attn, bw.lse, ws.delta, d_qkv, B, N, g.heads, g.dh)
         ev_last = None
-        if tr:
-            side = k.side_stream(main.device)
-            ev = torch.cuda.Event()
-            ev.record(main)
+
+        def side_section(ev):
+            nonlocal ev_last
             side.wait_event(ev)
             with torch.cuda.stream(side):
+                if top_side:
+                    if side_work is not None:
+                        side_work()
+                    if not last_bias_grad_done:
+                        k.colsum(dxc, gr["mlp.fc2.bias"], R, D)
+                    mlp_grads()
+                    k.layernorm_bwd_reduce([(tb["ws_ln"], nb, D, gr["norm2.weight"], gr["norm2.bias"], gr["attn.proj.bias"])])
+                    proj_grad()
                 k.colsum(d_qkv, gr["attn.qkv.bias"], M, 3 * D)
                 k.linear_wgrad(d_qkv, bw.ln1, gr["attn.qkv.weight"], M, 3 * D, D, acc("attn.qkv.weight"))
                 ev_last = torch.cuda.Event()
                 ev_last.record(side)
                 if on_block_done is not None:
                     on_block_done(i)
+
+        ev = None
+        if tr:
+            ev = torch.cuda.Event()
+            ev.record(main)
+            if not top_side:
+                side_section(ev)
         k.linear_dgrad(d_qkv, p["attn.qkv.weight"], ws.d_ln, M, 3 * D, D)
         k.layernorm_bwd(ws.d_ln, xin, p["norm1.weight"], bw.mean1, bw.rstd1, dmid, din, din_act, G_("norm1.weight"), G_("norm1.bias"),
                         below_bias, M, D)
+        if tr and top_side:
+            side_section(ev)
         if not tr and on_block_done is not None:
             on_block_done(i)
         return (ev_last,) if ev_last is not None else None
diff --git a/ssl4polyp_amd/models.py b/ssl4polyp_amd/models.py
--- a/ssl4polyp_amd/models.py
+++ b/ssl4polyp_amd/models.py
@@ -302,21 +302,28 @@
             dx = ws.dx[0] if below_head else None
             dx_act = ws.dx_act[0] if below_head else None
         x_rows = 1 if cls_top else (N if (below or pool) else 1)
-        _lib.check(k.lib.pm_vit_head_bwd(
-            _ptr(dout) if head else None, None if head else _ptr(dout), _ptr(x), x_rows, pool,
-            _ptr(f.param_view("norm.weight")), _ptr(f.param_view("lin_head.weight")) if head else None, _ptr(feat), _ptr(xhm),
-            _ptr(mean), _ptr(rstd), _ptr(dx), _ptr(dx_act), k.act,
-            _ptr(f.grad_view("lin_head.weight")) if need("lin_head.weight") else None,
-            _ptr(f.grad_view("lin_head.bias")) if need("lin_head.bias") else None,
-            _ptr(f.grad_view("norm.weight")) if need("norm.weight") else None,
-            _ptr(f.grad_view("norm.bias")) if need("norm.bias") else None, B, D, n_class, _stream()), "pm_vit_head_bwd")
+        pg = [_ptr(f.grad_view(n)) if need(n) else None for n in ("lin_head.weight", "lin_head.bias", "norm.weight", "norm.bias")]
+
+        def head_bwd(dx_, dx_act_, pgrads):
+            _lib.check(k.lib.pm_vit_head_bwd(
+                _ptr(dout) if head else None, None if head else _ptr(dout), _ptr(x), x_rows, pool,
+                _ptr(f.param_view("norm.weight")), _ptr(f.param_view("lin_head.weight")) if head else None, _ptr(feat), _ptr(xhm),
+                _ptr(mean), _ptr(rstd), _ptr(dx_), _ptr(dx_act_), k.act, *pgrads, B, D, n_class, _stream()), "pm_vit_head_bwd")
+
+        head_pgrads = None
+        if (k.TOP_SIDE and cls_top and below_head and trainable[-1] and any(v is not None for v in pg)
+                and not torch.cuda.is_current_stream_capturing()):
+            head_pgrads = lambda: head_bwd(None, None, pg)
+            head_bwd(dx, dx_act, [None] * 4)
+        else:
+            head_bwd(dx, dx_act, pg)
         sync = rt.grad_sync
         if below_head:
             W, G = rt.stack_weights("blocks.", g.depth)
             cb = (lambda i: sync.block_done("blocks.", i)) if sync is not None else None
             dx0, _ = BlockStack(k, g).backward(ws, x0, W, G, dx, dx_act, False, trainable, front,
                                                lambda n, i: accumulate, cb, defer_join=k.DEFER_JOIN,
-                                               sparse_top=True if cls_top else None)
+                                               sparse_top=True if cls_top else None, top_side_work=head_pgrads)
             if front and dx0 is not None:
                 _EncoderFrontMixin.front_bwd(rt, dx0, cols, None, B, L, accumulate, need, learn_pos)
             BlockStack.join_deferred(ws)
```

Measured after the change: 6395 images/sec (median of 6 runs). No clear change (+0.8%).
